# pixray/pixray

Hardware: AMD Instinct MI355X
Metric: optimisation iters/sec, VQGAN 256^2 + ViT-B/32 + 64 cutouts (higher is better)
Workload: dtype fp16

## Files before the change

pixray_amd/csrc/common.h:

```cpp
#pragma once
#include <hip/hip_runtime.h>
#include <stdint.h>

typedef __bf16 bf16_t;
typedef _Float16 half_t;
typedef __attribute__((ext_vector_type(8))) _Float16 f16x8;
typedef __attribute__((ext_vector_type(4))) _Float16 f16x4;
typedef __attribute__((ext_vector_type(8))) __bf16 bf16x8;
typedef __attribute__((ext_vector_type(4))) __bf16 bf16x4;
typedef __attribute__((ext_vector_type(2))) __bf16 bf16x2;
typedef __attribute__((ext_vector_type(16))) float f32x16;
typedef __attribute__((ext_vector_type(4))) float f32x4;

#define PRX_WAVE 64

enum { PRX_PREC_BF16 = 0, PRX_PREC_F32 = 1, PRX_PREC_F16 = 2 };
static inline int prec_is_f32(int precision) { return precision == PRX_PREC_F32; }
static inline int prec_is_h16(int precision) { return precision == PRX_PREC_F16; }
static inline bool prec_valid(int precision) { return precision >= PRX_PREC_BF16 && precision <= PRX_PREC_F16; }
static inline size_t op_esz(int f32) { return f32 ? 4 : 2; }
static inline void* op_off(void* p, size_t elems, int f32) { return p ? (char*)p + elems * op_esz(f32) : nullptr; }
static inline const void* op_off(const void* p, size_t elems, int f32) { return p ? (const char*)p + elems * op_esz(f32) : nullptr; }

void prx_set_error(const char* fmt, ...);
#define PRX_CHECK_HIP(expr)                                                        \
    do {                                                                           \
        hipError_t _e = (expr);                                                    \
        if (_e != hipSuccess) {                                                    \
            prx_set_error("%s:%d: %s -> %s", __FILE__, __LINE__, #expr,            \
                          hipGetErrorString(_e));                                  \
            return -1;                                                             \
        }                                                                          \
    } while (0)
#define PRX_REQUIRE(cond, ...)                                                     \
    do {                                                                           \
        if (!(cond)) {                                                             \
            prx_set_error(__VA_ARGS__);                                            \
            return -2;                                                             \
        }                                                                          \
    } while (0)
#define PRX_LAUNCH_CHECK()                                                         \
    do {                                                                           \
        hipError_t _e = hipGetLastError();                                         \
        if (_e != hipSuccess) {                                                    \
            prx_set_error("%s:%d: kernel launch -> %s", __FILE__, __LINE__,        \
                          hipGetErrorString(_e));                                  \
            return -1;                                                             \
        }                                                                          \
    } while (0)

__device__ __forceinline__ float bf16_to_f32(bf16_t v) { return (float)v; }
__device__ __forceinline__ bf16_t f32_to_bf16(float v) { return (bf16_t)v; }

__device__ __forceinline__ bf16x8 pack_bf16x8(const float* v) {
    bf16x8 r;
#pragma unroll
    for (int i = 0; i < 8; ++i) r[i] = (bf16_t)v[i];
    return r;
}

#define PRX_F16_MAX 65504.f
__device__ __forceinline__ half_t f32_to_f16_sat(float v) {
    return (half_t)__builtin_fminf(__builtin_fmaxf(v, -PRX_F16_MAX), PRX_F16_MAX);
}
__device__ __forceinline__ bf16_t to_op16(float v, int h16) {
    if (h16) return __builtin_bit_cast(bf16_t, f32_to_f16_sat(v));
    return (bf16_t)v;
}
__device__ __forceinline__ float from_op16(bf16_t b, int h16) {
    if (h16) return (float)__builtin_bit_cast(half_t, b);
    return (float)b;
}
__device__ __forceinline__ bf16x4 to_op16x4(float a, float b, float c, float d, int h16) {
    bf16x4 r;
    r[0] = to_op16(a, h16); r[1] = to_op16(b, h16); r[2] = to_op16(c, h16); r[3] = to_op16(d, h16);
    return r;
}

template <bool S16>
__device__ __forceinline__ float4 stream_ld4(const void* p, size_t i4, int h16) {
    if constexpr (S16) {
        const bf16x4 t = reinterpret_cast<const bf16x4*>(p)[i4];
        return make_float4(from_op16(t[0], h16), from_op16(t[1], h16), from_op16(t[2], h16), from_op16(t[3], h16));
    } else {
        return reinterpret_cast<const float4*>(p)[i4];
    }
}

template <typename T> __device__ __forceinline__ float op_ld(const T* p, size_t i) { return (float)p[i]; }
template <typename T> __device__ __forceinline__ void op_st(T* p, size_t i, float v) { p[i] = (T)v; }
template <typename T> __device__ __forceinline__ void op_ld4(const T* p, size_t i, float* v);
template <> __device__ __forceinline__ void op_ld4<bf16_t>(const bf16_t* p, size_t i, float* v) {
    const bf16x4 t = *reinterpret_cast<const bf16x4*>(p + i);
    v[0] = (float)t[0]; v[1] = (float)t[1]; v[2] = (float)t[2]; v[3] = (float)t[3];
}
template <> __device__ __forceinline__ void op_ld4<float>(const float* p, size_t i, float* v) {
    const float4 t = *reinterpret_cast<const float4*>(p + i);
    v[0] = t.x; v[1] = t.y; v[2] = t.z; v[3] = t.w;
}
template <> __device__ __forceinline__ void op_st<half_t>(half_t* p, size_t i, float v) { p[i] = f32_to_f16_sat(v); }
template <> __device__ __forceinline__ void op_ld4<half_t>(const half_t* p, size_t i, float* v) {
    const f16x4 t = *reinterpret_cast<const f16x4*>(p + i);
    v[0] = (float)t[0]; v[1] = (float)t[1]; v[2] = (float)t[2]; v[3] = (float)t[3];
}
template <typename T> __device__ __forceinline__ float4 op_ld4v(const T* p, size_t i);
template <> __device__ __forceinline__ float4 op_ld4v<bf16_t>(const bf16_t* p, size_t i) {
    const bf16x4 t = *reinterpret_cast<const bf16x4*>(p + i);
    return make_float4((float)t[0], (float)t[1], (float)t[2], (float)t[3]);
}
template <> __device__ __forceinline__ float4 op_ld4v<half_t>(const half_t* p, size_t i) {
    const f16x4 t = *reinterpret_cast<const f16x4*>(p + i);
    return make_float4((float)t[0], (float)t[1], (float)t[2], (float)t[3]);
}
template <> __device__ __forceinline__ float4 op_ld4v<float>(const float* p, size_t i) { return *reinterpret_cast<const float4*>(p + i); }
template <typename T> __device__ __forceinline__ void op_st4(T* p, size_t i, float a, float b, float c, float d);
template <> __device__ __forceinline__ void op_st4<half_t>(half_t* p, size_t i, float a, float b, float c, float d) {
    f16x4 r;
    r[0] = f32_to_f16_sat(a); r[1] = f32_to_f16_sat(b); r[2] = f32_to_f16_sat(c); r[3] = f32_to_f16_sat(d);
    *reinterpret_cast<f16x4*>(p + i) = r;
}
template <typename T> __device__ __forceinline__ T op_cvt(float v) { return (T)v; }
template <> __device__ __forceinline__ half_t op_cvt<half_t>(float v) { return f32_to_f16_sat(v); }

#define PRX_OP_DISPATCH(f32_, h16_, T, ...)                                   \
    do {                                                                      \
        if (f32_) { using T = float; __VA_ARGS__; }                           \
        else if (h16_) { using T = half_t; __VA_ARGS__; }                     \
        else { using T = bf16_t; __VA_ARGS__; }                               \
    } while (0)
template <> __device__ __forceinline__ void op_st4<bf16_t>(bf16_t* p, size_t i, float a, float b, float c, float d) {
    bf16x4 r;
    r[0] = (bf16_t)a; r[1] = (bf16_t)b; r[2] = (bf16_t)c; r[3] = (bf16_t)d;
    *reinterpret_cast<bf16x4*>(p + i) = r;
}
template <> __device__ __forceinline__ void op_st4<float>(float* p, size_t i, float a, float b, float c, float d) {
    *reinterpret_cast<float4*>(p + i) = make_float4(a, b, c, d);
}

__device__ __forceinline__ float wave_sum(float v) {
#pragma unroll
    for (int o = 32; o > 0; o >>= 1) v += __shfl_xor(v, o, 64);
    return v;
}
__device__ __forceinline__ float wave_max(float v) {
#pragma unroll
    for (int o = 32; o > 0; o >>= 1) v = fmaxf(v, __shfl_xor(v, o, 64));
    return v;
}
__device__ __forceinline__ float wave_min(float v) {
#pragma unroll
    for (int o = 32; o > 0; o >>= 1) v = fminf(v, __shfl_xor(v, o, 64));
    return v;
}
__device__ __forceinline__ double wave_sum_d(double v) {
#pragma unroll
    for (int o = 32; o > 0; o >>= 1) v += __shfl_xor(v, o, 64);
    return v;
}

__device__ __forceinline__ float sigmoidf_(float x) { return 1.f / (1.f + __expf(-x)); }

__device__ __forceinline__ unsigned xcd_linear(unsigned bid, unsigned nwg) {
    const unsigned xcd = bid & 7u, local = bid >> 3, q = nwg >> 3, r = nwg & 7u;
    return (xcd < r ? xcd * (q + 1) : r * (q + 1) + (xcd - r) * q) + local;
}
int prx_xcd_local();
int prx_grad_target_log2();

static inline int ceil_div(int a, int b) { return (a + b - 1) / b; }
static inline long long ceil_div_ll(long long a, long long b) { return (a + b - 1) / b; }
```

pixray_amd/csrc/elementwise.h:

```cpp
#pragma once
#include "common.h"
int prx_transpose_op(const void* in, int ldin, void* out, int ldout, int R, int C, int f32, hipStream_t s);
int prx_softmax_rows(const float* S, int lds_, float scale, void* P, int ldp, void* PT, int ldpt, int rows,
                     int cols, int prec, hipStream_t s);
int prx_softmax_rows_bwd(const void* P, int ldp, const float* dP, int lddp, float scale, void* dS, int ldds,
                         void* dST, int lddst, int rows, int cols, int prec, hipStream_t s);
int prx_upsample2x_bwd(const void* hi, float* low, bf16_t* low_bf16, int NB, int Hl, int Wl, int C, hipStream_t s, int h16 = 0, int s16 = 0);
int prx_nchw_to_nhwc(const float* in, float* out_f32, bf16_t* out_bf16, int NB, int C, int HW, int Cpad, hipStream_t s, int h16 = 0);
int prx_nhwc_to_nchw(const float* in, int ldc, float* out, int NB, int C, int HW, hipStream_t s);
int prx_image_head_fwd(const float* x, int ldc, float* img, int NB, int C, int HW, hipStream_t s);
int prx_image_head_bwd(const float* x, int ldc, const float* gimg, float* dx, bf16_t* dx_bf16, int ldo, int NB, int C,
                       int HW, hipStream_t s, int h16 = 0, const float* gscale = nullptr);
int prx_image_head_bwd_im2col(const float* x, int ldc, const float* gimg, bf16_t* col, int ldk, int C, int H, int W, hipStream_t s, int h16 = 0,
                              const float* gscale = nullptr);
int prx_grad_scale(const float* g, size_t n, float* part, int nparts, int target_log2, float* scale2, hipStream_t s);
int prx_adam_clamp(float* z, float* m, float* v, const float* g, const float* zmin, const float* zmax, int hw,
                   size_t n, float lr, float b1, float b2, float eps, int step, hipStream_t s);
int prx_adam_clamp_dev(float* z, float* m, float* v, const float* g, const float* zmin, const float* zmax, int hw,
                       size_t n, const float* hyper, float b1, float b2, float eps, hipStream_t s);
int prx_f32_to_bf16(const float* in, bf16_t* out, size_t n, hipStream_t s, int h16 = 0);
int prx_grad_scale_multi(const float* const* gs, const size_t* ns, int count, float* part, int nparts_each, int target_log2,
                         float* scale2, hipStream_t s);
int prx_add_f32(const float* a, const float* b, float* out, size_t n, hipStream_t s);
int prx_scale_dev(float* x, size_t n, const float* scale, hipStream_t s, bf16_t* out16 = nullptr, int h16 = 0);
```

pixray_amd/csrc/elementwise.hip:

```cpp
#include "elementwise.h"
#include <algorithm>

namespace {

inline int ew_grid(size_t total, int per = 256) { return (int)std::min<size_t>((total + per - 1) / per, 8192); }

template <typename T>
__global__ __launch_bounds__(256) void transpose_op_kernel(const T* __restrict__ in, int ldin,
                                                           T* __restrict__ out, int ldout, int R, int C) {
    __shared__ T tile[32][33];
    const int tx = threadIdx.x & 31, ty = threadIdx.x >> 5;
    const int r0 = blockIdx.y * 32, c0 = blockIdx.x * 32;
#pragma unroll
    for (int i = 0; i < 4; ++i) {
        int r = r0 + ty + 8 * i, c = c0 + tx;
        tile[ty + 8 * i][tx] = (r < R && c < C) ? in[(size_t)r * ldin + c] : (T)0.f;
    }
    __syncthreads();
#pragma unroll
    for (int i = 0; i < 4; ++i) {
        int c = c0 + ty + 8 * i, r = r0 + tx;
        if (c < C && r < R) out[(size_t)c * ldout + r] = tile[tx][ty + 8 * i];
    }
}

template <typename T>
__global__ __launch_bounds__(256) void softmax_rows_kernel(const float* __restrict__ S, int lds_, float scale,
                                                           T* __restrict__ P, int ldp, T* __restrict__ PT,
                                                           int ldpt, int rows, int cols) {
    const int lane = threadIdx.x & 63;
    const int row = blockIdx.x * 4 + (threadIdx.x >> 6);
    if (row >= rows) return;
    const float* s = S + (size_t)row * lds_;
    float mx = -INFINITY;
    for (int c = lane; c < cols; c += 64) mx = fmaxf(mx, s[c] * scale);
    mx = wave_max(mx);
    float sum = 0.f;
    for (int c = lane; c < cols; c += 64) sum += __expf(s[c] * scale - mx);
    sum = wave_sum(sum);
    const float inv = 1.f / sum;
    for (int c = lane; c < cols; c += 64) {
        T p = op_cvt<T>(__expf(s[c] * scale - mx) * inv);
        P[(size_t)row * ldp + c] = p;
        if (PT) PT[(size_t)c * ldpt + row] = p;
    }
}

template <typename T>
__global__ __launch_bounds__(256) void softmax_rows_bwd_kernel(const T* __restrict__ P, int ldp,
                                                               const float* __restrict__ dP, int lddp, float scale,
                                                               T* __restrict__ dS, int ldds,
                                                               T* __restrict__ dST, int lddst, int rows, int cols) {
    const int lane = threadIdx.x & 63;
    const int row = blockIdx.x * 4 + (threadIdx.x >> 6);
    if (row >= rows) return;
    float dot = 0.f;
    for (int c = lane; c < cols; c += 64)
        dot += (float)P[(size_t)row * ldp + c] * dP[(size_t)row * lddp + c];
    dot = wave_sum(dot);
    for (int c = lane; c < cols; c += 64) {
        float p = (float)P[(size_t)row * ldp + c];
        T v = op_cvt<T>(scale * p * (dP[(size_t)row * lddp + c] - dot));
        dS[(size_t)row * ldds + c] = v;
        if (dST) dST[(size_t)c * lddst + row] = v;
    }
}

template <bool S16>
__global__ __launch_bounds__(256) void upsample2x_bwd_kernel(const void* __restrict__ hi, float* __restrict__ low,
                                                             bf16_t* __restrict__ low_bf16, int NB, int Hl, int Wl,
                                                             int C, int h16) {
    const int C4 = C >> 2;
    const size_t total = (size_t)NB * Hl * Wl * C4;
    const int Wh = Wl * 2;
    for (size_t idx = (size_t)blockIdx.x * blockDim.x + threadIdx.x; idx < total;
         idx += (size_t)gridDim.x * blockDim.x) {
        int cq = (int)(idx % C4);
        size_t pix = idx / C4;
        int x = (int)(pix % Wl);
        size_t t = pix / Wl;
        int y = (int)(t % Hl);
        int b = (int)(t / Hl);
        size_t p00 = (((size_t)b * Hl * 2 + 2 * y) * Wh + 2 * x) * C4 + cq;
        float4 a = stream_ld4<S16>(hi, p00, h16), bb = stream_ld4<S16>(hi, p00 + C4, h16), c = stream_ld4<S16>(hi, p00 + (size_t)Wh * C4, h16),
               d = stream_ld4<S16>(hi, p00 + (size_t)Wh * C4 + C4, h16);
        float4 o = make_float4((a.x + bb.x) + (c.x + d.x), (a.y + bb.y) + (c.y + d.y), (a.z + bb.z) + (c.z + d.z),
                               (a.w + bb.w) + (c.w + d.w));
        if (low) reinterpret_cast<float4*>(low)[idx] = o;
        if (low_bf16) {
            reinterpret_cast<bf16x4*>(low_bf16)[idx] = to_op16x4(o.x, o.y, o.z, o.w, h16);
        }
    }
}

__global__ __launch_bounds__(256) void nchw_to_nhwc_kernel(const float* __restrict__ in, float* __restrict__ out_f32,
                                                           bf16_t* __restrict__ out_bf16, int NB, int C, int HW,
                                                           int Cpad, int h16) {
    const size_t total = (size_t)NB * HW * Cpad;
    for (size_t idx = (size_t)blockIdx.x * blockDim.x + threadIdx.x; idx < total;
         idx += (size_t)gridDim.x * blockDim.x) {
        int c = (int)(idx % Cpad);
        size_t t = idx / Cpad;
        int p = (int)(t % HW);
        int b = (int)(t / HW);
        float v = c < C ? in[((size_t)b * C + c) * HW + p] : 0.f;
        if (out_f32) out_f32[idx] = v;
        if (out_bf16) out_bf16[idx] = to_op16(v, h16);
    }
}

__global__ __launch_bounds__(256) void nhwc_to_nchw_kernel(const float* __restrict__ in, int ldc,
                                                           float* __restrict__ out, int NB, int C, int HW) {
    const size_t total = (size_t)NB * C * HW;
    for (size_t idx = (size_t)blockIdx.x * blockDim.x + threadIdx.x; idx < total;
         idx += (size_t)gridDim.x * blockDim.x) {
        int p = (int)(idx % HW);
        size_t t = idx / HW;
        int c = (int)(t % C);
        int b = (int)(t / C);
        out[idx] = in[((size_t)b * HW + p) * ldc + c];
    }
}

__global__ __launch_bounds__(256) void image_head_fwd_kernel(const float* __restrict__ x, int ldc,
                                                             float* __restrict__ img, int NB, int C, int HW) {
    const size_t total = (size_t)NB * C * HW;
    for (size_t idx = (size_t)blockIdx.x * blockDim.x + threadIdx.x; idx < total;
         idx += (size_t)gridDim.x * blockDim.x) {
        int p = (int)(idx % HW);
        size_t t = idx / HW;
        int c = (int)(t % C);
        int b = (int)(t / C);
        float v = (x[((size_t)b * HW + p) * ldc + c] + 1.f) * 0.5f;
        img[idx] = fminf(fmaxf(v, 0.f), 1.f);
    }
}

__global__ __launch_bounds__(256) void image_head_bwd_kernel(const float* __restrict__ x, int ldc,
                                                             const float* __restrict__ gimg, float* __restrict__ dx,
                                                             bf16_t* __restrict__ dx_bf16, int ldo, int NB, int C,
                                                             int HW, int h16, const float* __restrict__ gscale_dev) {
    const float gscale = gscale_dev ? *gscale_dev : 1.f;
    const size_t total = (size_t)NB * HW * ldo;
    for (size_t idx = (size_t)blockIdx.x * blockDim.x + threadIdx.x; idx < total;
         idx += (size_t)gridDim.x * blockDim.x) {
        int c = (int)(idx % ldo);
        size_t t = idx / ldo;
        int p = (int)(t % HW);
        int b = (int)(t / HW);
        float o = 0.f;
        if (c < C) {
            float u = (x[((size_t)b * HW + p) * ldc + c] + 1.f) * 0.5f;
            float g = gimg[((size_t)b * C + c) * HW + p];
            float uc = fminf(fmaxf(u, 0.f), 1.f);
            o = (g * (u - uc) >= 0.f) ? (0.5f * gscale) * g : 0.f;
        }
        if (dx) dx[idx] = o;
        if (dx_bf16) dx_bf16[idx] = to_op16(o, h16);
    }
}

__global__ __launch_bounds__(256) void image_head_bwd_im2col_kernel(const float* __restrict__ x, int ldc, const float* __restrict__ gimg,
                                                                    bf16_t* __restrict__ col, int ldk, int C, int H, int W, int h16,
                                                                    const float* __restrict__ gscale_dev) {
    const float gscale = gscale_dev ? *gscale_dev : 1.f;
    const int slots = ldk / 8;
    const size_t HW = (size_t)H * W, total = HW * slots;
    for (size_t idx = (size_t)blockIdx.x * blockDim.x + threadIdx.x; idx < total; idx += (size_t)gridDim.x * blockDim.x) {
        const int tap = (int)(idx % slots);
        const size_t p = idx / slots;
        const int py = (int)(p / W), px = (int)(p - (size_t)py * W);
        bf16x8 o;
#pragma unroll
        for (int c = 0; c < 8; ++c) o[c] = to_op16(0.f, h16);
        if (tap < 9) {
            const int yy = py + tap / 3 - 1, xx = px + tap % 3 - 1;
            if (yy >= 0 && yy < H && xx >= 0 && xx < W) {
                const size_t q = (size_t)yy * W + xx;
#pragma unroll
                for (int c = 0; c < 8; ++c) {
                    if (c < C) {
                        const float u = (x[q * ldc + c] + 1.f) * 0.5f;
                        const float g = gimg[(size_t)c * HW + q];
                        const float uc = fminf(fmaxf(u, 0.f), 1.f);
                        o[c] = to_op16((g * (u - uc) >= 0.f) ? (0.5f * gscale) * g : 0.f, h16);
                    }
                }
            }
        }
        reinterpret_cast<bf16x8*>(col)[idx] = o;
    }
}

__global__ __launch_bounds__(256) void adam_clamp_kernel(float* __restrict__ z, float* __restrict__ m,
                                                         float* __restrict__ v, const float* __restrict__ g,
                                                         const float* __restrict__ zmin, const float* __restrict__ zmax,
                                                         int hw, size_t n, float lr, float b1, float b2, float eps,
                                                         float bc1, float bc2_sqrt, const float* __restrict__ hyper) {
    if (hyper) { lr = hyper[0]; bc1 = 1.f; bc2_sqrt = hyper[1]; }
    for (size_t i = (size_t)blockIdx.x * blockDim.x + threadIdx.x; i < n; i += (size_t)gridDim.x * blockDim.x) {
        float gi = g[i];
        float mi = b1 * m[i] + (1.f - b1) * gi;
        float vi = b2 * v[i] + (1.f - b2) * gi * gi;
        m[i] = mi; v[i] = vi;
        float denom = sqrtf(vi) / bc2_sqrt + eps;
        float zi = z[i] - (lr / bc1) * (mi / denom);
        if (zmin) {
            int c = (int)(i / hw);
            zi = fminf(fmaxf(zi, zmin[c]), zmax[c]);
        }
        z[i] = zi;
    }
}

__global__ __launch_bounds__(256) void f32_to_bf16_kernel(const float* __restrict__ in, bf16_t* __restrict__ out,
                                                          size_t n, int h16) {
    for (size_t i = (size_t)blockIdx.x * blockDim.x + threadIdx.x; i < n; i += (size_t)gridDim.x * blockDim.x)
        out[i] = to_op16(in[i], h16);
}

__global__ __launch_bounds__(256) void amax_partial_kernel(const float* __restrict__ g, size_t n, float* __restrict__ part) {
    float m = 0.f;
    for (size_t i = (size_t)blockIdx.x * blockDim.x + threadIdx.x; i < n; i += (size_t)gridDim.x * blockDim.x) {
        const float a = fabsf(g[i]);
        m = fmaxf(m, a == a ? a : INFINITY);
    }
    m = wave_max(m);
    __shared__ float s[4];
    if ((threadIdx.x & 63) == 0) s[threadIdx.x >> 6] = m;
    __syncthreads();
    if (threadIdx.x == 0) part[blockIdx.x] = fmaxf(fmaxf(s[0], s[1]), fmaxf(s[2], s[3]));
}
__global__ __launch_bounds__(256) void grad_scale_final_kernel(const float* __restrict__ part, int nparts, int target_log2,
                                                               float* __restrict__ scale2) {
    float m = 0.f;
    for (int i = threadIdx.x; i < nparts; i += blockDim.x) m = fmaxf(m, part[i]);
    m = wave_max(m);
    __shared__ float s[4];
    if ((threadIdx.x & 63) == 0) s[threadIdx.x >> 6] = m;
    __syncthreads();
    if (threadIdx.x == 0) {
        m = fmaxf(fmaxf(s[0], s[1]), fmaxf(s[2], s[3]));
        float S = 1.f;
        if (m > 0.f && m < INFINITY) {
            int e;
            (void)frexpf(m, &e);
            int k = target_log2 - e;
            k = k < -40 ? -40 : (k > 60 ? 60 : k);
            S = ldexpf(1.f, k);
        }
        scale2[0] = S;
        scale2[1] = 1.f / S;
    }
}

__global__ __launch_bounds__(256) void scale_dev_kernel(float* __restrict__ x, size_t n, const float* __restrict__ scale, bf16_t* __restrict__ out16, int h16) {
    const float sc = *scale;
    for (size_t i = (size_t)blockIdx.x * blockDim.x + threadIdx.x; i < n; i += (size_t)gridDim.x * blockDim.x) {
        const float v = x[i] * sc;
        x[i] = v;
        if (out16) out16[i] = to_op16(v, h16);
    }
}

__global__ __launch_bounds__(256) void add_f32_kernel(const float* __restrict__ a, const float* __restrict__ b,
                                                      float* __restrict__ out, size_t n) {
    for (size_t i = (size_t)blockIdx.x * blockDim.x + threadIdx.x; i < n; i += (size_t)gridDim.x * blockDim.x)
        out[i] = a[i] + b[i];
}

}

int prx_transpose_op(const void* in, int ldin, void* out, int ldout, int R, int C, int f32, hipStream_t s) {
    dim3 grid(ceil_div(C, 32), ceil_div(R, 32));
    if (f32) hipLaunchKernelGGL(transpose_op_kernel<float>, grid, dim3(256), 0, s, (const float*)in, ldin, (float*)out, ldout, R, C);
    else     hipLaunchKernelGGL(transpose_op_kernel<bf16_t>, grid, dim3(256), 0, s, (const bf16_t*)in, ldin, (bf16_t*)out, ldout, R, C);
    PRX_LAUNCH_CHECK();
    return 0;
}
int prx_softmax_rows(const float* S, int lds_, float scale, void* P, int ldp, void* PT, int ldpt, int rows,
                     int cols, int prec, hipStream_t s) {
    PRX_OP_DISPATCH(prec_is_f32(prec), prec_is_h16(prec), T,
                    hipLaunchKernelGGL(softmax_rows_kernel<T>, dim3(ceil_div(rows, 4)), dim3(256), 0, s, S, lds_, scale, (T*)P, ldp,
                                       (T*)PT, ldpt, rows, cols));
    PRX_LAUNCH_CHECK();
    return 0;
}
int prx_softmax_rows_bwd(const void* P, int ldp, const float* dP, int lddp, float scale, void* dS, int ldds,
                         void* dST, int lddst, int rows, int cols, int prec, hipStream_t s) {
    PRX_OP_DISPATCH(prec_is_f32(prec), prec_is_h16(prec), T,
                    hipLaunchKernelGGL(softmax_rows_bwd_kernel<T>, dim3(ceil_div(rows, 4)), dim3(256), 0, s, (const T*)P, ldp, dP, lddp,
                                       scale, (T*)dS, ldds, (T*)dST, lddst, rows, cols));
    PRX_LAUNCH_CHECK();
    return 0;
}
int prx_upsample2x_bwd(const void* hi, float* low, bf16_t* low_bf16, int NB, int Hl, int Wl, int C, hipStream_t s, int h16, int s16) {
    PRX_REQUIRE(C % 4 == 0 && (low || low_bf16), "upsample2x_bwd: C %% 4 != 0, or no output");
    if (s16) hipLaunchKernelGGL(upsample2x_bwd_kernel<true>, dim3(ew_grid((size_t)NB * Hl * Wl * C / 4)), dim3(256), 0, s, hi, low, low_bf16,
                                NB, Hl, Wl, C, h16);
    else hipLaunchKernelGGL(upsample2x_bwd_kernel<false>, dim3(ew_grid((size_t)NB * Hl * Wl * C / 4)), dim3(256), 0, s, hi, low, low_bf16,
                            NB, Hl, Wl, C, h16);
    PRX_LAUNCH_CHECK();
    return 0;
}
int prx_nchw_to_nhwc(const float* in, float* out_f32, bf16_t* out_bf16, int NB, int C, int HW, int Cpad,
                     hipStream_t s, int h16) {
    hipLaunchKernelGGL(nchw_to_nhwc_kernel, dim3(ew_grid((size_t)NB * HW * Cpad)), dim3(256), 0, s, in, out_f32,
                       out_bf16, NB, C, HW, Cpad, h16);
    PRX_LAUNCH_CHECK();
    return 0;
}
int prx_nhwc_to_nchw(const float* in, int ldc, float* out, int NB, int C, int HW, hipStream_t s) {
    hipLaunchKernelGGL(nhwc_to_nchw_kernel, dim3(ew_grid((size_t)NB * HW * C)), dim3(256), 0, s, in, ldc, out, NB, C,
                       HW);
    PRX_LAUNCH_CHECK();
    return 0;
}
int prx_image_head_fwd(const float* x, int ldc, float* img, int NB, int C, int HW, hipStream_t s) {
    hipLaunchKernelGGL(image_head_fwd_kernel, dim3(ew_grid((size_t)NB * HW * C)), dim3(256), 0, s, x, ldc, img, NB, C,
                       HW);
    PRX_LAUNCH_CHECK();
    return 0;
}
int prx_grad_scale(const float* g, size_t n, float* part, int nparts, int target_log2, float* scale2, hipStream_t s) {
    PRX_REQUIRE(nparts >= 1 && nparts <= 1024, "grad_scale: 1..1024 partials");
    const int blocks = (int)std::min<size_t>((n + 1023) / 1024 + 1, (size_t)nparts);
    hipLaunchKernelGGL(amax_partial_kernel, dim3(blocks), dim3(256), 0, s, g, n, part);
    PRX_LAUNCH_CHECK();
    hipLaunchKernelGGL(grad_scale_final_kernel, dim3(1), dim3(256), 0, s, part, blocks, target_log2, scale2);
    PRX_LAUNCH_CHECK();
    return 0;
}
int prx_grad_scale_multi(const float* const* gs, const size_t* ns, int count, float* part, int nparts_each, int target_log2,
                         float* scale2, hipStream_t s) {
    PRX_REQUIRE(count >= 1 && nparts_each >= 1 && (long long)count * nparts_each <= 4096, "grad_scale_multi: bad partial layout");
    int used = 0;
    for (int i = 0; i < count; ++i) {
        if (!gs[i] || ns[i] == 0) continue;
        const int blocks = (int)std::min<size_t>((ns[i] + 1023) / 1024 + 1, (size_t)nparts_each);
        hipLaunchKernelGGL(amax_partial_kernel, dim3(blocks), dim3(256), 0, s, gs[i], ns[i], part + used);
        PRX_LAUNCH_CHECK();
        used += blocks;
    }
    PRX_REQUIRE(used > 0, "grad_scale_multi: no gradient tensor");
    hipLaunchKernelGGL(grad_scale_final_kernel, dim3(1), dim3(256), 0, s, part, used, target_log2, scale2);
    PRX_LAUNCH_CHECK();
    return 0;
}
int prx_scale_dev(float* x, size_t n, const float* scale, hipStream_t s, bf16_t* out16, int h16) {
    hipLaunchKernelGGL(scale_dev_kernel, dim3(ew_grid(n)), dim3(256), 0, s, x, n, scale, out16, h16);
    PRX_LAUNCH_CHECK();
    return 0;
}
int prx_image_head_bwd(const float* x, int ldc, const float* gimg, float* dx, bf16_t* dx_bf16, int ldo, int NB, int C,
                       int HW, hipStream_t s, int h16, const float* gscale) {
    hipLaunchKernelGGL(image_head_bwd_kernel, dim3(ew_grid((size_t)NB * HW * ldo)), dim3(256), 0, s, x, ldc, gimg, dx,
                       dx_bf16, ldo, NB, C, HW, h16, gscale);
    PRX_LAUNCH_CHECK();
    return 0;
}
int prx_image_head_bwd_im2col(const float* x, int ldc, const float* gimg, bf16_t* col, int ldk, int C, int H, int W, hipStream_t s, int h16,
                              const float* gscale) {
    PRX_REQUIRE(C <= 8 && ldk % 8 == 0 && ldk >= 72, "image_head_bwd_im2col: at most 8 channels, row pitch a multiple of 8 >= 72");
    hipLaunchKernelGGL(image_head_bwd_im2col_kernel, dim3(ew_grid((size_t)H * W * (ldk / 8))), dim3(256), 0, s, x, ldc, gimg, col, ldk, C, H, W,
                       h16, gscale);
    PRX_LAUNCH_CHECK();
    return 0;
}
int prx_adam_clamp(float* z, float* m, float* v, const float* g, const float* zmin, const float* zmax, int hw,
                   size_t n, float lr, float b1, float b2, float eps, int step, hipStream_t s) {
    PRX_REQUIRE(step >= 1, "adam: step must be >= 1");
    const double bc1 = 1.0 - pow((double)b1, step);
    const double bc2 = 1.0 - pow((double)b2, step);
    hipLaunchKernelGGL(adam_clamp_kernel, dim3(ew_grid(n)), dim3(256), 0, s, z, m, v, g, zmin, zmax, hw, n, lr, b1, b2,
                       eps, (float)bc1, (float)sqrt(bc2), (const float*)nullptr);
    PRX_LAUNCH_CHECK();
    return 0;
}
int prx_adam_clamp_dev(float* z, float* m, float* v, const float* g, const float* zmin, const float* zmax, int hw,
                       size_t n, const float* hyper, float b1, float b2, float eps, hipStream_t s) {
    PRX_REQUIRE(hyper != nullptr, "adam: null hyper buffer");
    hipLaunchKernelGGL(adam_clamp_kernel, dim3(ew_grid(n)), dim3(256), 0, s, z, m, v, g, zmin, zmax, hw, n, 0.f, b1, b2,
                       eps, 1.f, 1.f, hyper);
    PRX_LAUNCH_CHECK();
    return 0;
}
int prx_f32_to_bf16(const float* in, bf16_t* out, size_t n, hipStream_t s, int h16) {
    hipLaunchKernelGGL(f32_to_bf16_kernel, dim3(ew_grid(n)), dim3(256), 0, s, in, out, n, h16);
    PRX_LAUNCH_CHECK();
    return 0;
}
int prx_add_f32(const float* a, const float* b, float* out, size_t n, hipStream_t s) {
    hipLaunchKernelGGL(add_f32_kernel, dim3(ew_grid(n)), dim3(256), 0, s, a, b, out, n);
    PRX_LAUNCH_CHECK();
    return 0;
}
```

pixray_amd/csrc/resnet.hip:

```cpp
#include "resnet.h"
#include "gemm.h"
#include "attention.h"
#include "elementwise.h"
#include "cutouts.h"
#include "prompt_vq.h"
#include "vit.h"
#include "dev_arena.h"
#include <cstdlib>
#include <vector>
#include <memory>
#include <algorithm>

namespace {

__constant__ float r_clip_mean[3] = {0.48145466f, 0.4578275f, 0.40821073f};
__constant__ float r_clip_std[3] = {0.26862954f, 0.26130258f, 0.27577711f};

inline int rgrid(size_t total) { return (int)std::min<size_t>((total + 255) / 256, 16384); }

template <typename TOp>
__global__ __launch_bounds__(256) void rn_pack_conv3x3_kernel(const float* __restrict__ w, void* __restrict__ Wf_, void* __restrict__ Wd_,
                                                              int Cout, int Cin) {
    TOp* Wf = reinterpret_cast<TOp*>(Wf_);
    TOp* Wd = reinterpret_cast<TOp*>(Wd_);
    const size_t total = (size_t)Cout * 9 * Cin;
    for (size_t i = (size_t)blockIdx.x * blockDim.x + threadIdx.x; i < 2 * total; i += (size_t)gridDim.x * blockDim.x) {
        if (i < total) {
            const int ci = (int)(i % Cin), tap = (int)((i / Cin) % 9), co = (int)(i / ((size_t)9 * Cin));
            Wf[i] = op_cvt<TOp>(w[(((size_t)co * Cin + ci) * 3 + tap / 3) * 3 + tap % 3]);
        } else {
            const size_t j = i - total;
            const int co = (int)(j % Cout), tap = (int)((j / Cout) % 9), ci = (int)(j / ((size_t)9 * Cout));
            Wd[j] = op_cvt<TOp>(w[(((size_t)co * Cin + ci) * 3 + (2 - tap / 3)) * 3 + (2 - tap % 3)]);
        }
    }
}

template <typename TOp, int CO>
__global__ __launch_bounds__(256) void stem1_fwd_kernel(const float* __restrict__ cut, const float* __restrict__ mm,
                                                        const float* __restrict__ w, const float* __restrict__ b,
                                                        void* __restrict__ out_, int N, int S) {
    __shared__ __attribute__((aligned(16))) float ws[27 * CO];
    __shared__ float bs[CO];
    for (int i = threadIdx.x; i < 27 * CO; i += 256) {
        const int co = i % CO, t = i / CO;
        ws[i] = w[co * 27 + t];
    }
    for (int i = threadIdx.x; i < CO; i += 256) bs[i] = b[i];
    __syncthreads();
    TOp* out = reinterpret_cast<TOp*>(out_);
    const int So = S / 2;
    const float mn = mm[0], range = mm[1] - mm[0];
    const float inv = range != 0.f ? 1.f / range : 1.f;
    const size_t total = (size_t)N * So * So;
    constexpr bool STAGE = sizeof(TOp) == 2;
    __shared__ __attribute__((aligned(16))) TOp otile[STAGE ? 256 * CO : 4];
    for (size_t pixb = (size_t)blockIdx.x * blockDim.x; pixb < total; pixb += (size_t)gridDim.x * blockDim.x) {
        const size_t pix = pixb + threadIdx.x;
        if (pix < total) {
        const int xo = (int)(pix % So), yo = (int)((pix / So) % So), n = (int)(pix / ((size_t)So * So));
        float v[27];
#pragma unroll
        for (int c = 0; c < 3; ++c) {
            const float im = r_clip_mean[c], is = 1.f / r_clip_std[c];
#pragma unroll
            for (int ky = 0; ky < 3; ++ky)
#pragma unroll
                for (int kx = 0; kx < 3; ++kx) {
                    const int y = 2 * yo + ky - 1, x = 2 * xo + kx - 1, t = (c * 3 + ky) * 3 + kx;
                    const bool ok = y >= 0 && y < S && x >= 0 && x < S;
                    const int yc = y < 0 ? 0 : (y < S ? y : S - 1), xc = x < 0 ? 0 : (x < S ? x : S - 1);
                    const float raw = cut[(((size_t)n * 3 + c) * S + yc) * S + xc];
                    v[t] = ok ? ((raw - mn) * inv - im) * is : 0.f;
                }
        }
        TOp* orow = STAGE ? otile + threadIdx.x * CO : out + pix * CO;
#pragma unroll 1
        for (int c0 = 0; c0 < CO; c0 += 4) {
            float a[4] = {bs[c0], bs[c0 + 1], bs[c0 + 2], bs[c0 + 3]};
#pragma unroll
            for (int t = 0; t < 27; ++t) {
                const float4 w4 = *reinterpret_cast<const float4*>(&ws[t * CO + c0]);
                a[0] += v[t] * w4.x; a[1] += v[t] * w4.y; a[2] += v[t] * w4.z; a[3] += v[t] * w4.w;
            }
            op_st4(orow, (size_t)c0, fmaxf(a[0], 0.f), fmaxf(a[1], 0.f), fmaxf(a[2], 0.f), fmaxf(a[3], 0.f));
        }
        }
        if constexpr (STAGE) {
        __syncthreads();
        {
            const size_t pix0 = pixb;
            const size_t npix = total - pix0 < 256 ? total - pix0 : 256;
            const int pieces = (int)(npix * CO * sizeof(TOp) / 16);
            const float4* src = reinterpret_cast<const float4*>(otile);
            float4* dst = reinterpret_cast<float4*>(out + pix0 * CO);
            for (int i = threadIdx.x; i < pieces; i += 256) dst[i] = src[i];
        }
        __syncthreads();
        }
    }
}

template <typename TOp, int CO>
__global__ __launch_bounds__(256) void stem1_bwd_kernel(const void* __restrict__ g_, const float* __restrict__ w, float* __restrict__ dY,
                                                        int N, int S, const float* __restrict__ oscale_dev) {
    const float oscale = oscale_dev ? *oscale_dev : 1.f;
    __shared__ float ws[27 * CO];
    for (int i = threadIdx.x; i < 27 * CO; i += 256) {
        const int co = i % CO, c = (i / CO) % 3, kx = (i / (3 * CO)) % 3, ky = i / (9 * CO);
        ws[i] = w[((co * 3 + c) * 3 + ky) * 3 + kx];
    }
    __syncthreads();
    const TOp* g = reinterpret_cast<const TOp*>(g_);
    const int So = S / 2;
    const size_t plane = (size_t)S * S, total = (size_t)N * plane;
    for (size_t pix = (size_t)blockIdx.x * blockDim.x + threadIdx.x; pix < total; pix += (size_t)gridDim.x * blockDim.x) {
        const int x = (int)(pix % S), y = (int)((pix / S) % S), n = (int)(pix / plane);
        float acc[3] = {0.f, 0.f, 0.f};
        for (int ky = 0; ky < 3; ++ky) {
            const int t = y + 1 - ky;
            if (t < 0 || (t & 1)) continue;
            const int yo = t >> 1;
            if (yo >= So) continue;
            for (int kx = 0; kx < 3; ++kx) {
                const int u = x + 1 - kx;
                if (u < 0 || (u & 1)) continue;
                const int xo = u >> 1;
                if (xo >= So) continue;
                const TOp* gp = g + (((size_t)n * So + yo) * So + xo) * CO;
                const float* wp = ws + (ky * 3 + kx) * 3 * CO;
#pragma unroll
                for (int c0 = 0; c0 < CO; c0 += 4) {
                    float gv[4];
                    op_ld4(gp, (size_t)c0, gv);
#pragma unroll
                    for (int q = 0; q < 4; ++q) {
                        acc[0] += gv[q] * wp[c0 + q];
                        acc[1] += gv[q] * wp[CO + c0 + q];
                        acc[2] += gv[q] * wp[2 * CO + c0 + q];
                    }
                }
            }
        }
        float* o = dY + (size_t)n * 3 * plane + (size_t)y * S + x;
        o[0] = acc[0] * oscale; o[plane] = acc[1] * oscale; o[2 * plane] = acc[2] * oscale;
    }
}

template <typename TOp>
__global__ __launch_bounds__(256) void avgpool2_fwd_kernel(const void* __restrict__ x_, void* __restrict__ out_, int N, int H, int W, int C) {
    const TOp* x = reinterpret_cast<const TOp*>(x_);
    TOp* out = reinterpret_cast<TOp*>(out_);
    const int Ho = H / 2, Wo = W / 2, C4 = C / 4;
    const size_t total = (size_t)N * Ho * Wo * C4;
    for (size_t idx = (size_t)blockIdx.x * blockDim.x + threadIdx.x; idx < total; idx += (size_t)gridDim.x * blockDim.x) {
        const int c = (int)(idx % C4) * 4;
        const size_t pix = idx / C4;
        const int xo = (int)(pix % Wo), yo = (int)((pix / Wo) % Ho), n = (int)(pix / ((size_t)Ho * Wo));
        const size_t p = (((size_t)n * H + 2 * yo) * W + 2 * xo) * C + c;
        const float4 a = op_ld4v(x, p), b = op_ld4v(x, p + C), e = op_ld4v(x, p + (size_t)W * C), f = op_ld4v(x, p + (size_t)W * C + C);
        op_st4(out, pix * C + c, 0.25f * ((a.x + b.x) + (e.x + f.x)), 0.25f * ((a.y + b.y) + (e.y + f.y)),
               0.25f * ((a.z + b.z) + (e.z + f.z)), 0.25f * ((a.w + b.w) + (e.w + f.w)));
    }
}
template <typename TOp>
__global__ __launch_bounds__(256) void avgpool2_bwd_kernel(const float* __restrict__ g, const void* __restrict__ mask_,
                                                           float* __restrict__ dx_f32, void* __restrict__ dx_bf_, int N, int H, int W, int C) {
    const TOp* mask = reinterpret_cast<const TOp*>(mask_);
    TOp* dx_bf = reinterpret_cast<TOp*>(dx_bf_);
    const int Ho = H / 2, Wo = W / 2, C4 = C / 4;
    const size_t total = (size_t)N * Ho * Wo * C4;
    for (size_t idx = (size_t)blockIdx.x * blockDim.x + threadIdx.x; idx < total; idx += (size_t)gridDim.x * blockDim.x) {
        const int c = (int)(idx % C4) * 4;
        const size_t pix = idx / C4;
        const int xo = (int)(pix % Wo), yo = (int)((pix / Wo) % Ho), n = (int)(pix / ((size_t)Ho * Wo));
        float4 v = *reinterpret_cast<const float4*>(g + pix * C + c);
        v.x *= 0.25f; v.y *= 0.25f; v.z *= 0.25f; v.w *= 0.25f;
#pragma unroll
        for (int q = 0; q < 4; ++q) {
            const size_t o = (((size_t)n * H + 2 * yo + (q >> 1)) * W + 2 * xo + (q & 1)) * C + c;
            float4 u = v;
            if (mask) {
                const float4 m = op_ld4v(mask, o);
                if (!(m.x > 0.f)) u.x = 0.f;
                if (!(m.y > 0.f)) u.y = 0.f;
                if (!(m.z > 0.f)) u.z = 0.f;
                if (!(m.w > 0.f)) u.w = 0.f;
            }
            if (dx_f32) *reinterpret_cast<float4*>(dx_f32 + o) = u;
            if (dx_bf) op_st4(dx_bf, o, u.x, u.y, u.z, u.w);
        }
    }
}
template <typename TOp>
__global__ __launch_bounds__(256) void relu_mask_kernel(float* __restrict__ g, const void* __restrict__ out_, void* __restrict__ g_bf_, size_t n) {
    const TOp* out = reinterpret_cast<const TOp*>(out_);
    TOp* g_bf = reinterpret_cast<TOp*>(g_bf_);
    for (size_t i = (size_t)blockIdx.x * blockDim.x + threadIdx.x; i < n; i += (size_t)gridDim.x * blockDim.x) {
        const float v = ((float)out[i] > 0.f) ? g[i] : 0.f;
        g[i] = v;
        g_bf[i] = op_cvt<TOp>(v);
    }
}
template <typename TOp>
__global__ __launch_bounds__(256) void tokens_fwd_kernel(const float* __restrict__ x, const float* __restrict__ pos, void* __restrict__ t_,
                                                         int N, int P, int C) {
    TOp* t = reinterpret_cast<TOp*>(t_);
    const size_t total = (size_t)N * C;
    for (size_t idx = (size_t)blockIdx.x * blockDim.x + threadIdx.x; idx < total; idx += (size_t)gridDim.x * blockDim.x) {
        const int c = (int)(idx % C), n = (int)(idx / C);
        const float* xp = x + (size_t)n * P * C + c;
        TOp* tp = t + (size_t)n * (P + 1) * C + c;
        float sum = 0.f;
        for (int p = 0; p < P; ++p) {
            const float v = xp[(size_t)p * C];
            sum += v;
            tp[(size_t)(p + 1) * C] = op_cvt<TOp>(v + pos[(size_t)(p + 1) * C + c]);
        }
        tp[0] = op_cvt<TOp>(sum / (float)P + pos[c]);
    }
}
template <typename TOp>
__global__ __launch_bounds__(256) void tokens_bwd_kernel(const float* __restrict__ dt, float* __restrict__ dx, int N, int P, int C) {

    const size_t total = (size_t)N * P * C;
    const float ip = 1.f / (float)P;
    for (size_t idx = (size_t)blockIdx.x * blockDim.x + threadIdx.x; idx < total; idx += (size_t)gridDim.x * blockDim.x) {
        const int c = (int)(idx % C);
        const size_t np = idx / C;
        const int p = (int)(np % P), n = (int)(np / P);
        const float* base = dt + (size_t)n * (P + 1) * C + c;
        dx[idx] = base[(size_t)(p + 1) * C] + base[0] * ip;
    }
}
template <typename TOp>
__global__ __launch_bounds__(256) void tok0_gather_kernel(const void* __restrict__ t_, void* __restrict__ out_, int N, int T, int C) {
    const TOp* t = reinterpret_cast<const TOp*>(t_);
    TOp* out = reinterpret_cast<TOp*>(out_);
    const size_t total = (size_t)N * C;
    for (size_t idx = (size_t)blockIdx.x * blockDim.x + threadIdx.x; idx < total; idx += (size_t)gridDim.x * blockDim.x)
        out[idx] = t[(idx / C) * (size_t)T * C + idx % C];
}
template <typename TOp>
__global__ __launch_bounds__(256) void tok0_scatter_kernel(const void* __restrict__ g0_, void* __restrict__ dt_, int N, int T, int C) {
    const TOp* g0 = reinterpret_cast<const TOp*>(g0_);
    TOp* dt = reinterpret_cast<TOp*>(dt_);
    const size_t total = (size_t)N * T * C;
    for (size_t idx = (size_t)blockIdx.x * blockDim.x + threadIdx.x; idx < total; idx += (size_t)gridDim.x * blockDim.x) {
        const int c = (int)(idx % C);
        const size_t nt = idx / C;
        const int tok = (int)(nt % T), n = (int)(nt / T);
        dt[idx] = tok == 0 ? g0[(size_t)n * C + c] : (TOp)0.f;
    }
}

struct RConv1 { int Cin, Cout; void *W, *WT; float* b; };
struct RConv3 { int Cin, Cout; void *Wf, *Wd; float* b; };
struct RBlock {
    int Cin, planes, Hin, stride; bool has_ds;
    RConv1 c1, c3, ds; RConv3 c2;
    void *a1, *a2, *p2, *xp, *out_bf; float* out_f32;
    const void* xin_bf; const float* xin_f32;
};

}

#define RLAUNCH(prec, kernel, total, ...)                                                                                \
    do {                                                                                                                 \
        PRX_REQUIRE(prec_valid(prec), #kernel ": unknown precision %d", prec);                                           \
        PRX_OP_DISPATCH(prec_is_f32(prec), prec_is_h16(prec), TO_,                                                       \
                        hipLaunchKernelGGL(kernel<TO_>, dim3(rgrid(total)), dim3(256), 0, s, __VA_ARGS__));              \
        PRX_LAUNCH_CHECK();                                                                                              \
    } while (0)
#define STEM_CASE(prec, kernel, CO_, total, ...)                                                                         \
    case CO_:                                                                                                            \
        PRX_OP_DISPATCH(prec_is_f32(prec), prec_is_h16(prec), TO_,                                                       \
                        hipLaunchKernelGGL((kernel<TO_, CO_>), dim3(rgrid(total)), dim3(256), 0, s, __VA_ARGS__));       \
        break;
#define STEM_LAUNCH(prec, kernel, total, co, ...)                                                                        \
    do {                                                                                                                 \
        PRX_REQUIRE(prec_valid(prec), #kernel ": unknown precision %d", prec);                                           \
        switch (co) {                                                                                                    \
            STEM_CASE(prec, kernel, 8, total, __VA_ARGS__) STEM_CASE(prec, kernel, 16, total, __VA_ARGS__)               \
            STEM_CASE(prec, kernel, 32, total, __VA_ARGS__) STEM_CASE(prec, kernel, 40, total, __VA_ARGS__)              \
            STEM_CASE(prec, kernel, 48, total, __VA_ARGS__) STEM_CASE(prec, kernel, 64, total, __VA_ARGS__)              \
            default: PRX_REQUIRE(false, "resnet stem: width/2 = %d is not one of 8, 16, 32, 40, 48, 64", co);            \
        }                                                                                                                \
        PRX_LAUNCH_CHECK();                                                                                              \
    } while (0)

int prx_rn_pack_conv3x3(const float* w, void* Wf, void* Wd, int Cout, int Cin, int prec, hipStream_t s) {
    RLAUNCH(prec, rn_pack_conv3x3_kernel, (size_t)1024 * 256, w, Wf, Wd, Cout, Cin);
    return 0;
}
int prx_stem1_fwd(const float* cut, const float* mm, const float* w, const float* b, void* out, int N, int S, int CO, int prec,
                  hipStream_t s) {
    PRX_REQUIRE(N >= 1 && S >= 2, "resnet stem: %d cutouts of side %d", N, S);
    STEM_LAUNCH(prec, stem1_fwd_kernel, (size_t)N * (S / 2) * (S / 2), CO, cut, mm, w, b, out, N, S);
    return 0;
}
int prx_stem1_bwd(const void* g, const float* w, float* dY, int N, int S, int CO, const float* oscale_dev, int prec, hipStream_t s) {
    PRX_REQUIRE(N >= 1 && S >= 2, "resnet stem: %d cutouts of side %d", N, S);
    STEM_LAUNCH(prec, stem1_bwd_kernel, (size_t)N * S * S, CO, g, w, dY, N, S, oscale_dev);
    return 0;
}
int prx_avgpool2_fwd(const void* x, void* out, int N, int H, int W, int C, int prec, hipStream_t s) {
    PRX_REQUIRE(C % 4 == 0, "avgpool2: C = %d is not a multiple of 4", C);
    RLAUNCH(prec, avgpool2_fwd_kernel, (size_t)N * (H / 2) * (W / 2) * C / 4, x, out, N, H, W, C);
    return 0;
}
int prx_avgpool2_bwd(const float* g, const void* mask, float* dx_f32, void* dx_op, int N, int H, int W, int C, int prec, hipStream_t s) {
    PRX_REQUIRE(C % 4 == 0, "avgpool2: C = %d is not a multiple of 4", C);
    RLAUNCH(prec, avgpool2_bwd_kernel, (size_t)N * (H / 2) * (W / 2) * C / 4, g, mask, dx_f32, dx_op, N, H, W, C);
    return 0;
}
int prx_relu_mask(float* g, const void* out, void* g_op, size_t n, int prec, hipStream_t s) {
    RLAUNCH(prec, relu_mask_kernel, n, g, out, g_op, n);
    return 0;
}
int prx_tokens_fwd(const float* x, const float* pos, void* t, int N, int P, int C, int prec, hipStream_t s) {
    RLAUNCH(prec, tokens_fwd_kernel, (size_t)N * C, x, pos, t, N, P, C);
    return 0;
}
int prx_tokens_bwd(const float* dt, float* dx, int N, int P, int C, int prec, hipStream_t s) {
    RLAUNCH(prec, tokens_bwd_kernel, (size_t)N * P * C, dt, dx, N, P, C);
    return 0;
}
int prx_tok0_gather(const void* t, void* out, int N, int T, int C, int prec, hipStream_t s) {
    RLAUNCH(prec, tok0_gather_kernel, (size_t)N * C, t, out, N, T, C);
    return 0;
}
int prx_tok0_scatter(const void* g0, void* dt, int N, int T, int C, int prec, hipStream_t s) {
    RLAUNCH(prec, tok0_scatter_kernel, (size_t)N * T * C, g0, dt, N, T, C);
    return 0;
}

struct PrxResNet {
    int res, width, heads, out_dim, max_n, C, G, T, cur_n;
    int prec;
    int f32, h16;
    int lean;
    float* gs;
    GemmCtx gctx;
    DevArena mem;
    float *w1, *b1;
    RConv3 s2, s3;
    std::vector<RBlock> blocks;
    float* pos; void *Win, *WinT, *Wc, *WcT; float *bin, *bc;
    void *s1, *s2a, *s3a, *s0_bf; float* s0_f32;
    void *tok, *qkv, *att, *o0, *dtok, *dqkv, *do0; float *lse, *e, *de, *dtokf;
    float *gA, *gB, *tf; void *tb1, *tb2, *gbf;
    void *gb2, *gb3;
    float *dY, *mm_part, *ws; size_t ws_bytes;
};

namespace {
struct RCur { const float* const* w; int n, pos; };
#define RNEXT(cur, dst) do { PRX_REQUIRE((cur).pos < (cur).n, "resnet_create: weight list too short"); (dst) = (cur).w[(cur).pos++]; } while (0)

int mk1(PrxResNet* r, RConv1& c, int Cin, int Cout, RCur& cur, hipStream_t s) {
    const float *w, *b; RNEXT(cur, w); RNEXT(cur, b);
    c.Cin = Cin; c.Cout = Cout;
    DEV_ALLOC(r->mem, alloc_op, c.W, (size_t)Cout * Cin, r->f32); DEV_ALLOC(r->mem, alloc_op, c.WT, (size_t)Cout * Cin, r->f32);
    int e;
    if ((e = prx_pack_op(w, c.W, (size_t)Cout * Cin, r->prec, s))) return e;
    if ((e = prx_pack_transpose_op(w, c.WT, Cout, Cin, r->prec, s))) return e;
    return r->mem.copy_f32(&c.b, b, Cout, s);
}
int mk3(PrxResNet* r, RConv3& c, int Cin, int Cout, RCur& cur, hipStream_t s) {
    const float *w, *b; RNEXT(cur, w); RNEXT(cur, b);
    c.Cin = Cin; c.Cout = Cout;
    DEV_ALLOC(r->mem, alloc_op, c.Wf, (size_t)Cout * 9 * Cin, r->f32); DEV_ALLOC(r->mem, alloc_op, c.Wd, (size_t)Cout * 9 * Cin, r->f32);
    int e;
    if ((e = prx_rn_pack_conv3x3(w, c.Wf, c.Wd, Cout, Cin, r->prec, s))) return e;
    return r->mem.copy_f32(&c.b, b, Cout, s);
}
int rg(PrxResNet* r, GemmDesc& d, hipStream_t s) {
    if (r->f32) { d.f32 = 1; d.a_is_f32 = 0; }
    d.h16 = r->h16;
    return prx_gemm_launch(d, r->ws, r->ws_bytes, s, &r->gctx);
}

int lin(PrxResNet* r, const void* A, int M, int K, const void* Bt, int N, const float* bias, const float* resid, int act,
        const void* aux, float* of, void* ob, hipStream_t s, int resid16 = 0) {
    GemmDesc d; d.A = A; d.lda = K; d.B = Bt; d.ldb = K; d.M = M; d.N = N; d.K = K;
    d.bias_n = bias; d.resid = resid; d.ldr = N; d.act = act; d.aux = aux; d.ldaux = N; d.row16 = resid16 ? 1 : 0;
    d.out_f32 = of; d.ldc_f32 = N; d.out_bf16 = ob; d.ldc_bf16 = N;
    return rg(r, d, s);
}
int conv3(PrxResNet* r, const void* x, int NB, int H, int Cin, const void* Bt, int Cout, const float* bias, int act,
          const void* aux, float* of, void* ob, hipStream_t s) {
    GemmDesc d; d.A = x; d.a_mode = PRX_A_CONV3X3; d.lda = Cin; d.B = Bt; d.ldb = 9 * Cin; d.M = NB * H * H; d.N = Cout; d.K = 9 * Cin;
    d.H = H; d.W = H; d.Cin = Cin; d.bias_n = bias; d.act = act; d.aux = aux; d.ldaux = Cout;
    d.out_f32 = of; d.ldc_f32 = Cout; d.out_bf16 = ob; d.ldc_bf16 = Cout;
    return rg(r, d, s);
}
}

GemmCtx* prx_resnet_gemm_ctx_impl(PrxResNet* r) { return r ? &r->gctx : nullptr; }

int prx_resnet_create_impl(PrxResNet** out, int res, int width, const int* layers, int heads, int out_dim, int max_n,
                           int precision, const float* const* w, int n_w, hipStream_t s) {
    PRX_REQUIRE(prec_valid(precision), "resnet_create: unknown precision %d", precision);
    PRX_REQUIRE(res % 32 == 0 && width % 16 == 0 && max_n >= 1, "resnet_create: unsupported geometry (res %d width %d)", res, width);
    PRX_REQUIRE(width * 32 == heads * 64, "resnet_create: the attention pool needs head dim 64 (width %d heads %d)", width, heads);
    std::unique_ptr<PrxResNet> guard(new PrxResNet());
    PrxResNet* r = guard.get();
    DevArena& m = r->mem;
    const int f32 = prec_is_f32(precision);
    m.describe("resnet_create", ": the runner keeps one forward's activations for max_batch = %d cutouts of %d x %d (width %d)", max_n, res, res,
               width);
    r->prec = precision; r->f32 = prec_is_f32(precision); r->h16 = prec_is_h16(precision);
    r->gs = nullptr;
    { const char* ev = getenv("PRX_RN_LEAN"); r->lean = (r->h16 && !(ev && atoi(ev) == 0)) ? 1 : 0; }
    r->res = res; r->width = width; r->heads = heads; r->out_dim = out_dim; r->max_n = max_n; r->cur_n = 0;
    r->C = width * 32; r->G = res / 32; r->T = r->G * r->G + 1;
    RCur cur{w, n_w, 0};
    int e;
    {   const float *ww, *bb; RNEXT(cur, ww); RNEXT(cur, bb);
        if ((e = m.copy_f32(&r->w1, ww, (size_t)(width / 2) * 27, s))) return e;
        if ((e = m.copy_f32(&r->b1, bb, width / 2, s))) return e; }
    if ((e = mk3(r, r->s2, width / 2, width / 2, cur, s))) return e;
    if ((e = mk3(r, r->s3, width / 2, width, cur, s))) return e;
    const size_t N = (size_t)max_n;
    int H = res / 4, inplanes = width;
    size_t maxMC = N * (size_t)(res / 2) * (res / 2) * width;
    for (int li = 0; li < 4; ++li) {
        const int planes = width << li;
        for (int b = 0; b < layers[li]; ++b) {
            RBlock k{};
            k.Cin = inplanes; k.planes = planes; k.Hin = H; k.stride = (li > 0 && b == 0) ? 2 : 1;
            k.has_ds = k.stride > 1 || inplanes != planes * 4;
            if ((e = mk1(r, k.c1, inplanes, planes, cur, s))) return e;
            if ((e = mk3(r, k.c2, planes, planes, cur, s))) return e;
            if ((e = mk1(r, k.c3, planes, planes * 4, cur, s))) return e;
            if (k.has_ds && (e = mk1(r, k.ds, inplanes, planes * 4, cur, s))) return e;
            const size_t Min = N * H * H, Ho = H / k.stride, Mout = N * Ho * Ho;
            DEV_ALLOC(m, alloc_op, k.a1, Min * planes, f32); DEV_ALLOC(m, alloc_op, k.a2, Min * planes, f32);
            k.p2 = k.a2; k.xp = nullptr;
            if (k.stride > 1) { DEV_ALLOC(m, alloc_op, k.p2, Mout * planes, f32); DEV_ALLOC(m, alloc_op, k.xp, Mout * inplanes, f32); }
            DEV_ALLOC(m, alloc_op, k.out_bf, Mout * planes * 4, f32);
            k.out_f32 = nullptr;
            if (!r->lean || (li == 3 && b == layers[li] - 1)) DEV_ALLOC(m, alloc, k.out_f32, Mout * planes * 4);
            maxMC = std::max(maxMC, std::max(Min * (size_t)std::max(inplanes, planes), Mout * (size_t)planes * 4));
            r->blocks.push_back(k);
            inplanes = planes * 4; H = (int)Ho;
        }
    }
    PRX_REQUIRE(inplanes == r->C && H == r->G, "resnet_create: internal geometry mismatch");
    const float *pos, *win, *bin, *wc, *bc;
    RNEXT(cur, pos); RNEXT(cur, win); RNEXT(cur, bin); RNEXT(cur, wc); RNEXT(cur, bc);
    PRX_REQUIRE(cur.pos == n_w, "resnet_create: %d weight tensors given, %d consumed", n_w, cur.pos);
    const int C = r->C, T = r->T;
    if ((e = m.copy_f32(&r->pos, pos, (size_t)T * C, s))) return e;
    DEV_ALLOC(m, alloc_op, r->Win, (size_t)3 * C * C, f32); DEV_ALLOC(m, alloc_op, r->WinT, (size_t)3 * C * C, f32);
    if ((e = prx_pack_op(win, r->Win, (size_t)3 * C * C, r->prec, s))) return e;
    if ((e = prx_pack_transpose_op(win, r->WinT, 3 * C, C, r->prec, s))) return e;
    if ((e = m.copy_f32(&r->bin, bin, 3 * C, s))) return e;
    DEV_ALLOC(m, alloc_op, r->Wc, (size_t)out_dim * C, f32); DEV_ALLOC(m, alloc_op, r->WcT, (size_t)out_dim * C, f32);
    if ((e = prx_pack_op(wc, r->Wc, (size_t)out_dim * C, r->prec, s))) return e;
    if ((e = prx_pack_transpose_op(wc, r->WcT, out_dim, C, r->prec, s))) return e;
    if ((e = m.copy_f32(&r->bc, bc, out_dim, s))) return e;
    const size_t S2 = (size_t)(res / 2) * (res / 2), S4 = (size_t)(res / 4) * (res / 4);
    DEV_ALLOC(m, alloc_op, r->s1, N * S2 * (width / 2), f32); DEV_ALLOC(m, alloc_op, r->s2a, N * S2 * (width / 2), f32);
    DEV_ALLOC(m, alloc_op, r->s3a, N * S2 * width, f32);
    DEV_ALLOC(m, alloc_op, r->s0_bf, N * S4 * width, f32); DEV_ALLOC(m, alloc, r->s0_f32, N * S4 * width);
    DEV_ALLOC(m, alloc_op, r->tok, N * T * C, f32); DEV_ALLOC(m, alloc_op, r->qkv, N * T * 3 * C, f32);
    DEV_ALLOC(m, alloc_op, r->att, N * T * C, f32); DEV_ALLOC(m, alloc_op, r->o0, N * C, f32);
    DEV_ALLOC(m, alloc_op, r->dtok, N * T * C, f32); DEV_ALLOC(m, alloc_op, r->dqkv, N * T * 3 * C, f32); DEV_ALLOC(m, alloc_op, r->do0, N * C, f32);
    DEV_ALLOC(m, alloc, r->dtokf, N * T * C);
    DEV_ALLOC(m, alloc, r->lse, N * heads * T); DEV_ALLOC(m, alloc, r->e, N * out_dim); DEV_ALLOC(m, alloc, r->de, N * out_dim);
    DEV_ALLOC(m, alloc, r->gA, maxMC); DEV_ALLOC(m, alloc, r->tf, maxMC);
    r->gB = nullptr; r->gb2 = r->gb3 = nullptr;
    if (r->lean) { DEV_ALLOC(m, alloc_op, r->gb2, maxMC, f32); DEV_ALLOC(m, alloc_op, r->gb3, maxMC, f32); } else DEV_ALLOC(m, alloc, r->gB, maxMC);
    DEV_ALLOC(m, alloc_op, r->tb1, maxMC, f32); DEV_ALLOC(m, alloc_op, r->tb2, maxMC, f32); DEV_ALLOC(m, alloc_op, r->gbf, maxMC, f32);
    DEV_ALLOC(m, alloc, r->dY, N * 3 * (size_t)res * res); DEV_ALLOC(m, alloc, r->mm_part, 2 * 1024);
    if (r->h16) DEV_ALLOC(m, alloc, r->gs, 2 + 64);
    r->ws_bytes = (size_t)64 << 20;
    DEV_ALLOC(m, alloc, r->ws, r->ws_bytes / sizeof(float));
    *out = guard.release();
    return 0;
}

void prx_resnet_destroy_impl(PrxResNet* r) { delete r; }

int prx_resnet_minmax_impl(PrxResNet* r, const float* cutouts, int n, float* mm, hipStream_t s) {
    PRX_REQUIRE(n >= 1 && n <= r->max_n, "resnet: batch %d exceeds handle capacity %d", n, r->max_n);
    return prx_minmax(cutouts, (size_t)n * 3 * r->res * r->res, r->mm_part, 1024, mm, s);
}

int prx_resnet_forward_impl(PrxResNet* r, const float* cutouts, int n, const float* mm, float* embeds, hipStream_t s) {
    PRX_REQUIRE(n >= 1 && n <= r->max_n, "resnet: batch %d exceeds handle capacity %d", n, r->max_n);
    const int S = r->res, S2 = S / 2, S4 = S / 4, w = r->width, wh = w / 2;
    int e;
    r->cur_n = n;
    if ((e = prx_stem1_fwd(cutouts, mm, r->w1, r->b1, r->s1, n, S, wh, r->prec, s))) return e;
    if ((e = conv3(r, r->s1, n, S2, wh, r->s2.Wf, wh, r->s2.b, PRX_ACT_RELU, nullptr, nullptr, r->s2a, s))) return e;
    if ((e = conv3(r, r->s2a, n, S2, wh, r->s3.Wf, w, r->s3.b, PRX_ACT_RELU, nullptr, nullptr, r->s3a, s))) return e;
    if ((e = prx_avgpool2_fwd(r->s3a, r->s0_bf, n, S2, S2, w, r->prec, s))) return e;
    const void* x_bf = r->s0_bf; const float* x_f32 = nullptr;
    const int lean = r->lean;
    for (RBlock& k : r->blocks) {
        const int H = k.Hin, Ho = H / k.stride, Min = n * H * H, Mout = n * Ho * Ho, p = k.planes;
        k.xin_bf = x_bf; k.xin_f32 = x_f32;
        if ((e = lin(r, x_bf, Min, k.Cin, k.c1.W, p, k.c1.b, nullptr, PRX_ACT_RELU, nullptr, nullptr, k.a1, s))) return e;
        if ((e = conv3(r, k.a1, n, H, p, k.c2.Wf, p, k.c2.b, PRX_ACT_RELU, nullptr, nullptr, k.a2, s))) return e;
        if (k.stride > 1) {
            if ((e = prx_avgpool2_fwd(k.a2, k.p2, n, H, H, p, r->prec, s))) return e;
        }
        const float* idn = lean ? (const float*)x_bf : x_f32;
        if (k.has_ds) {
            const void* xi = x_bf;
            if (k.stride > 1) {
                if ((e = prx_avgpool2_fwd(x_bf, k.xp, n, H, H, k.Cin, r->prec, s))) return e;
                xi = k.xp;
            }
            if ((e = lin(r, xi, Mout, k.Cin, k.ds.W, 4 * p, k.ds.b, nullptr, PRX_ACT_NONE, nullptr, lean ? nullptr : r->tf,
                         lean ? r->tb1 : nullptr, s))) return e;
            idn = lean ? (const float*)r->tb1 : r->tf;
        }
        PRX_REQUIRE(idn != nullptr, "resnet: identity path without an fp32 input");
        if ((e = lin(r, k.p2, Mout, p, k.c3.W, 4 * p, k.c3.b, idn, PRX_ACT_RELU, nullptr, k.out_f32, k.out_bf, s, lean))) return e;
        x_bf = k.out_bf; x_f32 = k.out_f32;
    }
    const int C = r->C, T = r->T, P = T - 1;
    if ((e = prx_tokens_fwd(x_f32, r->pos, r->tok, n, P, C, r->prec, s))) return e;
    if ((e = lin(r, r->tok, n * T, C, r->Win, 3 * C, r->bin, nullptr, PRX_ACT_NONE, nullptr, nullptr, r->qkv, s))) return e;
    if (r->f32) { if ((e = prx_mha_fwd_f32((const float*)r->qkv, (float*)r->att, r->lse, n, T, C, r->heads, s))) return e; }
    else if ((e = prx_mha_fwd_gen((const bf16_t*)r->qkv, (bf16_t*)r->att, r->lse, n, T, C, r->heads, s, r->h16))) return e;
    if ((e = prx_tok0_gather(r->att, r->o0, n, T, C, r->prec, s))) return e;
    if ((e = lin(r, r->o0, n, C, r->Wc, r->out_dim, r->bc, nullptr, PRX_ACT_NONE, nullptr, r->e, nullptr, s))) return e;
    return prx_l2norm_fwd(r->e, embeds, n, r->out_dim, s);
}

int prx_resnet_backward_a_impl(PrxResNet* r, const float* cutouts, const float* mm, const float* d_embeds, double* acc,
                               hipStream_t s) {
    const int n = r->cur_n;
    PRX_REQUIRE(n >= 1, "resnet backward: no forward in flight on this handle");
    const int C = r->C, T = r->T, P = T - 1;
    int e;
    if ((e = prx_l2norm_bwd(r->e, d_embeds, r->de, n, r->out_dim, s))) return e;
    {   GemmDesc d; d.A = r->de; d.a_is_f32 = 1; d.lda = r->out_dim; d.B = r->WcT; d.ldb = r->out_dim; d.M = n; d.N = C; d.K = r->out_dim;
        d.out_bf16 = r->do0; d.ldc_bf16 = C;
        if (r->h16) {
            if ((e = prx_grad_scale(r->de, (size_t)n * r->out_dim, r->gs + 2, 64, prx_grad_target_log2(), r->gs, s))) return e;
            if ((e = prx_scale_dev(r->de, (size_t)n * r->out_dim, r->gs, s))) return e;
        }
        if ((e = rg(r, d, s))) return e; }
    if ((e = prx_tok0_scatter(r->do0, r->dtok, n, T, C, r->prec, s))) return e;
    if (r->f32) { if ((e = prx_mha_bwd_f32((const float*)r->qkv, (const float*)r->att, (const float*)r->dtok, r->lse, (float*)r->dqkv, n, T, C, r->heads, s))) return e; }
    else if ((e = prx_mha_bwd_gen((const bf16_t*)r->qkv, (const bf16_t*)r->att, (const bf16_t*)r->dtok, r->lse, (bf16_t*)r->dqkv, n, T, C, r->heads, s, r->h16))) return e;
    if ((e = lin(r, r->dqkv, n * T, 3 * C, r->WinT, C, nullptr, nullptr, PRX_ACT_NONE, nullptr, r->dtokf, nullptr, s))) return e;
    float* g = r->gA; float* g2 = r->gB;
    const int lean = r->lean;
    void* gb = r->gbf; void* gb_alt = r->gb2;
    if ((e = prx_tokens_bwd(r->dtokf, g, n, P, C, r->prec, s))) return e;
    for (int bi = (int)r->blocks.size() - 1; bi >= 0; --bi) {
        RBlock& k = r->blocks[bi];
        const int H = k.Hin, Ho = H / k.stride, Min = n * H * H, Mout = n * Ho * Ho, p = k.planes;
        if (bi == (int)r->blocks.size() - 1 && (e = prx_relu_mask(g, k.out_bf, gb, (size_t)Mout * 4 * p, r->prec, s))) return e;
        if (k.stride > 1) {
            if ((e = lin(r, gb, Mout, 4 * p, k.c3.WT, p, nullptr, nullptr, PRX_ACT_NONE, nullptr, r->tf, nullptr, s))) return e;
            if ((e = prx_avgpool2_bwd(r->tf, k.a2, nullptr, r->tb1, n, H, H, p, r->prec, s))) return e;
        } else {
            if ((e = lin(r, gb, Mout, 4 * p, k.c3.WT, p, nullptr, nullptr, PRX_ACT_MUL_RELUMASK, k.a2, nullptr, r->tb1, s))) return e;
        }
        if ((e = conv3(r, r->tb1, n, H, p, k.c2.Wd, p, nullptr, PRX_ACT_MUL_RELUMASK, k.a1, nullptr, r->tb2, s))) return e;
        const float* gid = lean ? (const float*)gb : g;
        if (k.has_ds) {
            if (k.stride > 1) {
                if ((e = lin(r, gb, Mout, 4 * p, k.ds.WT, k.Cin, nullptr, nullptr, PRX_ACT_NONE, nullptr, r->tf, nullptr, s))) return e;
                if ((e = prx_avgpool2_bwd(r->tf, nullptr, lean ? (float*)nullptr : g2, lean ? r->gb3 : (void*)nullptr, n, H, H, k.Cin,
                                          r->prec, s))) return e;
                gid = lean ? (const float*)r->gb3 : g2;
            } else {
                if ((e = lin(r, gb, Mout, 4 * p, k.ds.WT, k.Cin, nullptr, nullptr, PRX_ACT_NONE, nullptr, lean ? nullptr : r->tf,
                             lean ? r->gb3 : nullptr, s))) return e;
                gid = lean ? (const float*)r->gb3 : r->tf;
            }
        }
        if (lean) {
            if (bi > 0) {
                if ((e = lin(r, r->tb2, Min, p, k.c1.WT, k.Cin, nullptr, gid, PRX_ACT_RELUMASK_POST, r->blocks[bi - 1].out_bf, nullptr,
                             gb_alt, s, 1))) return e;
                std::swap(gb, gb_alt);
            } else if ((e = lin(r, r->tb2, Min, p, k.c1.WT, k.Cin, nullptr, gid, PRX_ACT_NONE, nullptr, g, nullptr, s, 1))) return e;
            continue;
        }
        float* dst = (gid == g2) ? g : g2;
        if (gid == r->tf) dst = g2;
        if (bi > 0) {
            if ((e = lin(r, r->tb2, Min, p, k.c1.WT, k.Cin, nullptr, gid, PRX_ACT_RELUMASK_POST, r->blocks[bi - 1].out_bf, dst, gb, s))) return e;
        } else if ((e = lin(r, r->tb2, Min, p, k.c1.WT, k.Cin, nullptr, gid, PRX_ACT_NONE, nullptr, dst, nullptr, s))) return e;
        if (dst != g) std::swap(g, g2);
    }
    const int S = r->res, S2 = S / 2, w = r->width, wh = w / 2;
    if ((e = prx_avgpool2_bwd(g, r->s3a, nullptr, r->tb1, n, S2, S2, w, r->prec, s))) return e;
    if ((e = conv3(r, r->tb1, n, S2, w, r->s3.Wd, wh, nullptr, PRX_ACT_MUL_RELUMASK, r->s2a, nullptr, r->tb2, s))) return e;
    if ((e = conv3(r, r->tb2, n, S2, wh, r->s2.Wd, wh, nullptr, PRX_ACT_MUL_RELUMASK, r->s1, nullptr, r->tb1, s))) return e;
    if ((e = prx_stem1_bwd(r->tb1, r->w1, r->dY, n, S, wh, r->h16 ? r->gs + 1 : nullptr, r->prec, s))) return e;
    return prx_preproc_bwd_reduce(cutouts, mm, r->dY, acc, n, S, s);
}

int prx_resnet_backward_b_impl(PrxResNet* r, const float* cutouts, const float* mm, const double* acc, float* g_cutouts,
                               hipStream_t s) {
    PRX_REQUIRE(r->cur_n >= 1, "resnet backward: no forward in flight on this handle");
    return prx_preproc_bwd_apply(cutouts, mm, r->dY, acc, g_cutouts, r->cur_n, r->res, s);
}
```

pixray_amd/csrc/vit.hip:

```cpp
#include "vit.h"
#include <stdlib.h>
#include "gemm.h"
#include "norms.h"
#include "attention.h"
#include "cutouts.h"
#include "prompt_vq.h"
#include "elementwise.h"
#include "dev_arena.h"
#include <vector>
#include <memory>

namespace {

template <typename TOp>
__global__ __launch_bounds__(256) void pack_transpose_kernel(const float* __restrict__ in, TOp* __restrict__ out,
                                                             int R, int C) {
    __shared__ float tile[32][33];
    const int tx = threadIdx.x & 31, ty = threadIdx.x >> 5;
    const int r0 = blockIdx.y * 32, c0 = blockIdx.x * 32;
#pragma unroll
    for (int i = 0; i < 4; ++i) {
        int r = r0 + ty + 8 * i, c = c0 + tx;
        tile[ty + 8 * i][tx] = (r < R && c < C) ? in[(size_t)r * C + c] : 0.f;
    }
    __syncthreads();
#pragma unroll
    for (int i = 0; i < 4; ++i) {
        int c = c0 + ty + 8 * i, r = r0 + tx;
        if (c < C && r < R) out[(size_t)c * R + r] = op_cvt<TOp>(tile[tx][ty + 8 * i]);
    }
}

__global__ __launch_bounds__(256) void add_cls_pos_kernel(float* __restrict__ x, const float* __restrict__ cls,
                                                          const float* __restrict__ pos, int N, int T, int W) {
    const size_t total = (size_t)N * T * W;
    for (size_t i = (size_t)blockIdx.x * blockDim.x + threadIdx.x; i < total; i += (size_t)gridDim.x * blockDim.x) {
        const int c = (int)(i % W);
        const int t = (int)((i / W) % T);
        float v = x[i] + pos[(size_t)t * W + c];
        if (t == 0) v += cls[c];
        x[i] = v;
    }
}

template <typename TOut>
__global__ __launch_bounds__(256) void embed_tokens_kernel(const float* __restrict__ x, const float* __restrict__ cls,
                                                           const float* __restrict__ pos, TOut* __restrict__ out, int N, int T, int W) {
    const size_t total = (size_t)N * T * W;
    for (size_t i = (size_t)blockIdx.x * blockDim.x + threadIdx.x; i < total; i += (size_t)gridDim.x * blockDim.x) {
        const int c = (int)(i % W);
        const int t = (int)((i / W) % T);
        const float p = pos[(size_t)t * W + c];
        op_st(out, i, t == 0 ? cls[c] + p : x[i] + p);
    }
}

__global__ __launch_bounds__(256) void scale_f32_kernel(float* __restrict__ x, size_t n, float s) {
    for (size_t i = (size_t)blockIdx.x * blockDim.x + threadIdx.x; i < n; i += (size_t)gridDim.x * blockDim.x) x[i] *= s;
}

template <bool BWD>
__global__ __launch_bounds__(256) void gelu_f32_kernel(const float* __restrict__ t, float* __restrict__ io, size_t n) {
    for (size_t i = (size_t)blockIdx.x * blockDim.x + threadIdx.x; i < n; i += (size_t)gridDim.x * blockDim.x) {
        const float x = t[i];
        const float cdf = 0.5f * (1.f + erff(x * 0.70710678f));
        if (BWD) io[i] *= cdf + x * (0.39894228f * expf(-0.5f * x * x));
        else io[i] = x * cdf;
    }
}

}

int prx_pack_op(const float* in, void* out, size_t n, int prec, hipStream_t s) {
    if (!prec_is_f32(prec)) return prx_f32_to_bf16(in, (bf16_t*)out, n, s, prec_is_h16(prec));
    PRX_CHECK_HIP(hipMemcpyAsync(out, in, n * sizeof(float), hipMemcpyDeviceToDevice, s));
    return 0;
}
int prx_pack_transpose_op(const float* in, void* out, int R, int C, int prec, hipStream_t s) {
    const dim3 grid(ceil_div(C, 32), ceil_div(R, 32));
    PRX_OP_DISPATCH(prec_is_f32(prec), prec_is_h16(prec), TO,
                    hipLaunchKernelGGL(pack_transpose_kernel<TO>, grid, dim3(256), 0, s, in, (TO*)out, R, C));
    PRX_LAUNCH_CHECK();
    return 0;
}
int prx_pack_bf16(const float* in, bf16_t* out, size_t n, hipStream_t s) { return prx_pack_op(in, out, n, 0, s); }
int prx_pack_transpose_bf16(const float* in, bf16_t* out, int R, int C, hipStream_t s) { return prx_pack_transpose_op(in, out, R, C, 0, s); }
int prx_vit_add_cls_pos(float* x, const float* cls, const float* pos, int N, int T, int W, hipStream_t s) {
    hipLaunchKernelGGL(add_cls_pos_kernel, dim3(2048), dim3(256), 0, s, x, cls, pos, N, T, W);
    PRX_LAUNCH_CHECK();
    return 0;
}
int prx_vit_embed_tokens(const float* x, const float* cls, const float* pos, void* out, int out16, int N, int T, int W, hipStream_t s) {
    if (out16) hipLaunchKernelGGL(embed_tokens_kernel<half_t>, dim3(2048), dim3(256), 0, s, x, cls, pos, (half_t*)out, N, T, W);
    else hipLaunchKernelGGL(embed_tokens_kernel<float>, dim3(2048), dim3(256), 0, s, x, cls, pos, (float*)out, N, T, W);
    PRX_LAUNCH_CHECK();
    return 0;
}
int prx_vit_gelu_f32(const float* t, float* io, size_t n, int bwd, hipStream_t s) {
    if (bwd) hipLaunchKernelGGL(gelu_f32_kernel<true>, dim3(2048), dim3(256), 0, s, t, io, n);
    else hipLaunchKernelGGL(gelu_f32_kernel<false>, dim3(2048), dim3(256), 0, s, t, io, n);
    PRX_LAUNCH_CHECK();
    return 0;
}
int prx_vit_scale_f32(float* x, size_t n, float scale, int blocks, hipStream_t s) {
    PRX_REQUIRE(blocks >= 1, "scale_f32: %d workgroups", blocks);
    hipLaunchKernelGGL(scale_f32_kernel, dim3(blocks), dim3(256), 0, s, x, n, scale);
    PRX_LAUNCH_CHECK();
    return 0;
}

struct VitLayer {
    float *ln1_g, *ln1_b, *bqkv, *bo, *ln2_g, *ln2_b, *b1, *b2;
    void *Wqkv, *WqkvT, *Wo, *WoT, *W1, *W1T, *W2, *W2T;
    void *x_in, *x_mid;
    float *mean1, *rstd1, *mean2, *rstd2;
    void *qkv, *t;
    void* o_save;
    float* lse;
};

struct PrxVit {
    int res, patch, width, layers, heads, out_dim, T, max_n, KP;
    int hd, aw;
    int prec;
    int f32, h16;
    float* gs;
    GemmCtx gctx;
    DevArena mem;
    void *Wp, *WpT, *projT, *proj;
    float *cls, *pos, *lnpre_g, *lnpre_b, *lnpost_g, *lnpost_b;
    std::vector<VitLayer> L;
    void *A0, *h, *att_o, *u, *hpost, *dt, *do_, *dqkv, *dx_bf, *dh_bf, *de16;
    float *xpre, *mean_pre, *rstd_pre, *mean_post, *rstd_post, *e, *dx, *dh, *dA0, *de, *dhpost, *mm_part;
    void* x_final;
    int lean;
    VitFamily fam;
    float* bp;
    int cls_tail;
    float* ws; size_t ws_bytes;
    int cur_n;
};

namespace {
int pack_both(PrxVit* v, void** W, void** WT, const float* src, int out, int in, hipStream_t s) {
    DEV_ALLOC(v->mem, alloc_op, *W, (size_t)out * in, v->f32);
    DEV_ALLOC(v->mem, alloc_op, *WT, (size_t)out * in, v->f32);
    int r = prx_pack_op(src, *W, (size_t)out * in, v->prec, s);
    if (r) return r;
    return prx_pack_transpose_op(src, *WT, out, in, v->prec, s);
}
}

VitFamily prx_vit_family_clip() {
    VitFamily f;
    f.patch_bias = 0; f.ln_pre = 1; f.eps = 1e-5f; f.act = PRX_ACT_QUICKGELU; f.dact = PRX_ACT_MUL_DQUICKGELU;
    f.norm = prx_patch_norm_clip(); f.head_dim = 64;
    return f;
}

int prx_vit_create_impl(PrxVit** out, int res, int patch, int width, int layers, int heads, int out_dim, int max_n,
                        int precision, const float* const* w, int n_w, hipStream_t s, const VitFamily* family) {
    const VitFamily fam = family ? *family : prx_vit_family_clip();
    const int n_head = 3 + (fam.patch_bias ? 1 : 0) + (fam.ln_pre ? 2 : 0);
    PRX_REQUIRE(prec_valid(precision), "vit_create: unknown precision %d", precision);
    PRX_REQUIRE(n_w == n_head + 12 * layers + 3, "vit_create: expected %d weight tensors, got %d", n_head + 12 * layers + 3, n_w);
    const int hd = fam.head_dim > 0 ? fam.head_dim : 64;
    PRX_REQUIRE(res % patch == 0 && width == heads * hd && width % 128 == 0 && (hd == 64 || hd == 32 || hd == 16),
                "vit_create: unsupported geometry (width %d, %d heads of %d)", width, heads, hd);
    PRX_REQUIRE(fam.ln_pre || layers >= 1, "vit_create: a tower without ln_pre needs at least one block");
    PRX_REQUIRE(fam.eps > 0.f && fam.norm.std[0] > 0.f && fam.norm.std[1] > 0.f && fam.norm.std[2] > 0.f,
                "vit_create: LayerNorm eps and the channel std must be positive");
    const int G = res / patch;
    const int T = G * G + 1;
    std::unique_ptr<PrxVit> guard(new PrxVit());
    PrxVit* v = guard.get();
    DevArena& m = v->mem;
    const int f32 = prec_is_f32(precision);
    v->mem.describe("vit_create", ": the runner keeps one forward's activations for max_batch = %d cutouts of %d tokens (width %d, %d layers)",
                    max_n, T, width, layers);
    v->T = T; v->max_n = max_n;
    v->res = res; v->patch = patch; v->width = width; v->layers = layers; v->heads = heads; v->out_dim = out_dim;
    v->prec = precision; v->f32 = prec_is_f32(precision); v->h16 = prec_is_h16(precision);
    v->gs = nullptr; v->fam = fam; v->bp = nullptr; v->hd = hd; v->aw = heads * 64;
    const int AW = v->aw;
    float *pad_w = nullptr, *pad_b = nullptr;
    if (hd != 64) {
        DEV_ALLOC(m, alloc, pad_w, (size_t)3 * AW * width);
        DEV_ALLOC(m, alloc, pad_b, (size_t)3 * AW);
    }
    { const char* e = getenv("PRX_LEAN"); v->lean = (v->h16 && !(e && atoi(e) == 0)) ? 1 : 0; }
    { const char* e = getenv("PRX_VIT_CLS_TAIL"); v->cls_tail = (e && atoi(e) == 0) ? 0 : 1; }
    v->T = T; v->max_n = max_n; v->KP = (3 * patch * patch + 7) / 8 * 8; v->cur_n = 0;
    const int W = width, KP = v->KP;
    int r;
    {
        const int K0 = 3 * patch * patch;
        float* padded;
        DEV_ALLOC(m, alloc, padded, (size_t)W * KP);
        PRX_CHECK_HIP(hipMemsetAsync(padded, 0, sizeof(float) * (size_t)W * KP, s));
        PRX_CHECK_HIP(hipMemcpy2DAsync(padded, sizeof(float) * KP, w[0], sizeof(float) * K0, sizeof(float) * K0, W,
                                       hipMemcpyDeviceToDevice, s));
        if ((r = pack_both(v, &v->Wp, &v->WpT, padded, W, KP, s))) return r;
    }
    const float* const* wh = w + 1;
    if (fam.patch_bias) { if ((r = v->mem.copy_f32(&v->bp, *wh++, W, s))) return r; }
    if ((r = v->mem.copy_f32(&v->cls, *wh++, W, s))) return r;
    if ((r = v->mem.copy_f32(&v->pos, *wh++, (size_t)T * W, s))) return r;
    v->lnpre_g = v->lnpre_b = nullptr;
    if (fam.ln_pre) {
        if ((r = v->mem.copy_f32(&v->lnpre_g, *wh++, W, s))) return r;
        if ((r = v->mem.copy_f32(&v->lnpre_b, *wh++, W, s))) return r;
    }
    v->L.resize(layers);
    const size_t R = (size_t)max_n * T;
    for (int l = 0; l < layers; ++l) {
        const float* const* q = w + n_head + 12 * l;
        VitLayer& y = v->L[l];
        if ((r = v->mem.copy_f32(&y.ln1_g, q[0], W, s))) return r;
        if ((r = v->mem.copy_f32(&y.ln1_b, q[1], W, s))) return r;
        if (hd == 64) {
            if ((r = pack_both(v, &y.Wqkv, &y.WqkvT, q[2], 3 * W, W, s))) return r;
            if ((r = v->mem.copy_f32(&y.bqkv, q[3], 3 * W, s))) return r;
            if ((r = pack_both(v, &y.Wo, &y.WoT, q[4], W, W, s))) return r;
        } else {
            const float qs = sqrtf(64.f / (float)hd);
            PRX_CHECK_HIP(hipMemsetAsync(pad_w, 0, sizeof(float) * (size_t)3 * AW * W, s));
            PRX_CHECK_HIP(hipMemsetAsync(pad_b, 0, sizeof(float) * (size_t)3 * AW, s));
            for (int sect = 0; sect < 3; ++sect) {
                PRX_CHECK_HIP(hipMemcpy2DAsync(pad_w + (size_t)sect * AW * W, sizeof(float) * 64 * W, q[2] + (size_t)sect * W * W, sizeof(float) * hd * W,
                                               sizeof(float) * hd * W, heads, hipMemcpyDeviceToDevice, s));
                PRX_CHECK_HIP(hipMemcpy2DAsync(pad_b + (size_t)sect * AW, sizeof(float) * 64, q[3] + (size_t)sect * W, sizeof(float) * hd,
                                               sizeof(float) * hd, heads, hipMemcpyDeviceToDevice, s));
            }
            if ((r = prx_vit_scale_f32(pad_w, (size_t)AW * W, qs, 256, s))) return r;
            if ((r = prx_vit_scale_f32(pad_b, (size_t)AW, qs, 1, s))) return r;
            if ((r = pack_both(v, &y.Wqkv, &y.WqkvT, pad_w, 3 * AW, W, s))) return r;
            if ((r = v->mem.copy_f32(&y.bqkv, pad_b, 3 * AW, s))) return r;
            PRX_CHECK_HIP(hipMemsetAsync(pad_w, 0, sizeof(float) * (size_t)W * AW, s));
            PRX_CHECK_HIP(hipMemcpy2DAsync(pad_w, sizeof(float) * 64, q[4], sizeof(float) * hd, sizeof(float) * hd, (size_t)W * heads,
                                           hipMemcpyDeviceToDevice, s));
            if ((r = pack_both(v, &y.Wo, &y.WoT, pad_w, W, AW, s))) return r;
        }
        if ((r = v->mem.copy_f32(&y.bo, q[5], W, s))) return r;
        if ((r = v->mem.copy_f32(&y.ln2_g, q[6], W, s))) return r;
        if ((r = v->mem.copy_f32(&y.ln2_b, q[7], W, s))) return r;
        if ((r = pack_both(v, &y.W1, &y.W1T, q[8], 4 * W, W, s))) return r;
        if ((r = v->mem.copy_f32(&y.b1, q[9], 4 * W, s))) return r;
        if ((r = pack_both(v, &y.W2, &y.W2T, q[10], W, 4 * W, s))) return r;
        if ((r = v->mem.copy_f32(&y.b2, q[11], W, s))) return r;
        if (v->lean) { DEV_ALLOC(m, alloc_op, y.x_in, R * W, f32); DEV_ALLOC(m, alloc_op, y.x_mid, R * W, f32); }
        else { float *a_, *b_; DEV_ALLOC(m, alloc, a_, R * W); DEV_ALLOC(m, alloc, b_, R * W); y.x_in = a_; y.x_mid = b_; }
        DEV_ALLOC(m, alloc, y.mean1, R); DEV_ALLOC(m, alloc, y.rstd1, R); DEV_ALLOC(m, alloc, y.mean2, R); DEV_ALLOC(m, alloc, y.rstd2, R);
        DEV_ALLOC(m, alloc_op, y.qkv, R * 3 * AW, f32); DEV_ALLOC(m, alloc_op, y.t, R * 4 * W, f32);
        y.o_save = nullptr; y.lse = nullptr;
        if (T > 64 || v->f32) { DEV_ALLOC(m, alloc_op, y.o_save, R * AW, f32); DEV_ALLOC(m, alloc, y.lse, (size_t)max_n * heads * T); }
    }
    const float* const* q = w + n_head + 12 * layers;
    if ((r = v->mem.copy_f32(&v->lnpost_g, q[0], W, s))) return r;
    if ((r = v->mem.copy_f32(&v->lnpost_b, q[1], W, s))) return r;
    if ((r = pack_both(v, &v->proj, &v->projT, q[2], W, out_dim, s))) return r;
    DEV_ALLOC(m, alloc_op, v->A0, R * KP, f32); DEV_ALLOC(m, alloc_op, v->h, R * W, f32);
    DEV_ALLOC(m, alloc_op, v->att_o, R * AW, f32); DEV_ALLOC(m, alloc_op, v->u, R * 4 * W, f32);
    DEV_ALLOC(m, alloc_op, v->hpost, (size_t)max_n * W, f32); DEV_ALLOC(m, alloc_op, v->de16, (size_t)max_n * out_dim, f32);
    DEV_ALLOC(m, alloc_op, v->dt, R * 4 * W, f32); DEV_ALLOC(m, alloc_op, v->do_, R * AW, f32); DEV_ALLOC(m, alloc_op, v->dqkv, R * 3 * AW, f32);
    DEV_ALLOC(m, alloc, v->xpre, R * W); DEV_ALLOC(m, alloc, v->mean_pre, R); DEV_ALLOC(m, alloc, v->rstd_pre, R);
    if (v->lean) DEV_ALLOC(m, alloc_op, v->x_final, R * W, f32);
    else { float* a_; DEV_ALLOC(m, alloc, a_, R * W); v->x_final = a_; }
    DEV_ALLOC(m, alloc, v->mean_post, max_n); DEV_ALLOC(m, alloc, v->rstd_post, max_n); DEV_ALLOC(m, alloc, v->e, (size_t)max_n * out_dim);
    v->dx = v->dh = nullptr;
    if (!v->lean) { DEV_ALLOC(m, alloc, v->dx, R * W); DEV_ALLOC(m, alloc, v->dh, R * W); }
    DEV_ALLOC(m, alloc, v->dA0, R * KP); DEV_ALLOC(m, alloc, v->de, (size_t)max_n * out_dim);
    if (v->f32) { v->dx_bf = v->dx; v->dh_bf = v->dh; }
    else { DEV_ALLOC(m, alloc_op, v->dx_bf, R * W, f32); DEV_ALLOC(m, alloc_op, v->dh_bf, R * W, f32); }
    DEV_ALLOC(m, alloc, v->dhpost, (size_t)max_n * W); DEV_ALLOC(m, alloc, v->mm_part, 2 * 1024);
    if (v->h16) DEV_ALLOC(m, alloc, v->gs, 2 + 64);
    v->ws_bytes = (size_t)64 << 20;
    DEV_ALLOC(m, alloc, v->ws, v->ws_bytes / sizeof(float));
    *out = guard.release();
    return 0;
}

void prx_vit_destroy_impl(PrxVit* v) { delete v; }

static int vit_gemm(PrxVit* v, GemmDesc& d, hipStream_t s) {
    if (v->f32) { d.f32 = 1; d.a_is_f32 = 0; }
    d.h16 = v->h16;
    return prx_gemm_launch(d, v->ws, v->ws_bytes, s, &v->gctx);
}
GemmCtx* prx_vit_gemm_ctx_impl(PrxVit* v) { return v ? &v->gctx : nullptr; }
long long prx_vit_debug_dqkv_impl(PrxVit* v, void* dst, long long max_bytes, hipStream_t s) {
    if (!v || v->cur_n < 1) return -1;
    const long long bytes = (long long)op_esz(v->f32) * v->cur_n * v->T * 3 * v->aw;
    if (bytes > max_bytes || hipMemcpyAsync(dst, v->dqkv, bytes, hipMemcpyDeviceToDevice, s) != hipSuccess) return -1;
    return bytes;
}

static int ln_op(PrxVit* v, const void* x, long long ldx, const float* g, const float* b, void* out, float* mean, float* rstd,
                 int rows, hipStream_t s) {
    return prx_layernorm_fwd(x, ldx, g, b, v->f32 ? nullptr : (bf16_t*)out, v->f32 ? (float*)out : nullptr, mean, rstd, rows,
                             v->width, v->fam.eps, s, v->h16, v->lean, 1);
}
static int ln_bwd_op(PrxVit* v, const void* g, long long ldg, const void* x, long long ldx, const float* gamma, const float* mean,
                     const float* rstd, const void* add, long long ldadd, float* dx, long long lddx, void* dx_op, int rows,
                     hipStream_t s, int add_every = 0, int s16 = 0) {
    return prx_layernorm_bwd(g, ldg, x, ldx, gamma, mean, rstd, add, ldadd, dx, lddx, v->f32 ? nullptr : (bf16_t*)dx_op, lddx, rows,
                             v->width, s, v->h16, add_every, s16, 1);
}

int prx_vit_minmax_impl(PrxVit* v, const float* cutouts, int n, float* mm, hipStream_t s) {
    PRX_REQUIRE(n >= 1 && n <= v->max_n, "vit: batch %d exceeds handle capacity %d", n, v->max_n);
    return prx_minmax(cutouts, (size_t)n * 3 * v->res * v->res, v->mm_part, 1024, mm, s);
}

int prx_vit_forward_impl(PrxVit* v, const float* cutouts, int n, const float* mm, float* embeds, hipStream_t s) {
    PRX_REQUIRE(n >= 1 && n <= v->max_n, "vit: batch %d exceeds handle capacity %d", n, v->max_n);
    const int W = v->width, T = v->T, R = n * T, KP = v->KP, AW = v->aw;
    int r;
    v->cur_n = n;
    if ((r = prx_patchify_fwd(cutouts, mm, v->A0, v->prec, n, v->res, v->patch, T, s, v->fam.norm))) return r;
    {
        GemmDesc d; d.A = v->A0; d.lda = KP; d.B = v->Wp; d.ldb = KP; d.M = R; d.N = W; d.K = KP;
        d.bias_n = v->bp;
        d.out_f32 = v->xpre; d.ldc_f32 = W;
        if ((r = vit_gemm(v, d, s))) return r;
    }
    const int lean = v->lean;
    void* x0 = v->layers > 0 ? v->L[0].x_in : v->x_final;
    if (v->fam.ln_pre) {
        if ((r = prx_vit_add_cls_pos(v->xpre, v->cls, v->pos, n, T, W, s))) return r;
        if ((r = prx_layernorm_fwd(v->xpre, W, v->lnpre_g, v->lnpre_b, lean ? (bf16_t*)x0 : nullptr, lean ? nullptr : (float*)x0, v->mean_pre,
                                   v->rstd_pre, R, W, v->fam.eps, s, v->h16, 0, 1))) return r;
    } else {
        if ((r = prx_vit_embed_tokens(v->xpre, v->cls, v->pos, x0, lean, n, T, W, s))) return r;
    }
    for (int l = 0; l < v->layers; ++l) {
        VitLayer& y = v->L[l];
        void* x_next = (l + 1 < v->layers) ? v->L[l + 1].x_in : v->x_final;
        if ((r = ln_op(v, y.x_in, W, y.ln1_g, y.ln1_b, v->h, y.mean1, y.rstd1, R, s))) return r;
        {   GemmDesc d; d.A = v->h; d.lda = W; d.B = y.Wqkv; d.ldb = W; d.M = R; d.N = 3 * AW; d.K = W;
            d.bias_n = y.bqkv; d.out_bf16 = y.qkv; d.ldc_bf16 = 3 * AW;
            if ((r = vit_gemm(v, d, s))) return r; }
        const void* att = v->att_o;
        if (v->f32) { if ((r = prx_mha_fwd_f32((const float*)y.qkv, (float*)y.o_save, y.lse, n, T, AW, v->heads, s))) return r; att = y.o_save; }
        else if (T <= 64) { if ((r = prx_mha_fwd((const bf16_t*)y.qkv, (bf16_t*)v->att_o, n, T, AW, v->heads, s, v->h16))) return r; }
        else { if ((r = prx_mha_fwd_gen((const bf16_t*)y.qkv, (bf16_t*)y.o_save, y.lse, n, T, AW, v->heads, s, v->h16))) return r; att = y.o_save; }
        const bool tail = v->cls_tail && l == v->layers - 1;
        const int rows = tail ? n : R;
        const int ldt = tail ? T * W : W;
        {   GemmDesc d; d.A = att; d.lda = tail ? T * AW : AW; d.B = y.Wo; d.ldb = AW; d.M = rows; d.N = W; d.K = AW;
            d.bias_n = y.bo; d.ldr = ldt;
            if (lean) { d.resid = (const float*)y.x_in; d.row16 = 1; d.out_bf16 = y.x_mid; d.ldc_bf16 = ldt; }
            else { d.resid = (const float*)y.x_in; d.out_f32 = (float*)y.x_mid; d.ldc_f32 = ldt; }
            if ((r = vit_gemm(v, d, s))) return r; }
        if ((r = ln_op(v, y.x_mid, ldt, y.ln2_g, y.ln2_b, v->h, y.mean2, y.rstd2, rows, s))) return r;
        {   GemmDesc d; d.A = v->h; d.lda = W; d.B = y.W1; d.ldb = W; d.M = rows; d.N = 4 * W; d.K = W;
            d.bias_n = y.b1; d.act = v->fam.act; d.out_bf16 = v->u; d.out_bf16_pre = y.t; d.ldc_bf16 = 4 * W;
            const bool own_pass = v->f32 && v->fam.act == PRX_ACT_GELU;
            if (own_pass) { d.act = PRX_ACT_NONE; d.out_bf16 = y.t; d.out_bf16_pre = nullptr; }
            if ((r = vit_gemm(v, d, s))) return r;
            if (own_pass) {
                if ((r = prx_vit_gelu_f32((const float*)y.t, (float*)v->u, (size_t)rows * 4 * W, 0, s))) return r;
            } }
        {   GemmDesc d; d.A = v->u; d.lda = 4 * W; d.B = y.W2; d.ldb = 4 * W; d.M = rows; d.N = W; d.K = 4 * W;
            d.bias_n = y.b2; d.ldr = ldt;
            if (lean) { d.resid = (const float*)y.x_mid; d.row16 = 1; d.out_bf16 = x_next; d.ldc_bf16 = ldt; }
            else { d.resid = (const float*)y.x_mid; d.out_f32 = (float*)x_next; d.ldc_f32 = ldt; }
            if ((r = vit_gemm(v, d, s))) return r; }
    }
    if ((r = ln_op(v, v->x_final, (long long)T * W, v->lnpost_g, v->lnpost_b, v->hpost, v->mean_post, v->rstd_post, n, s))) return r;
    {   GemmDesc d; d.A = v->hpost; d.lda = W; d.B = v->projT; d.ldb = W; d.M = n; d.N = v->out_dim; d.K = W;
        d.out_f32 = v->e; d.ldc_f32 = v->out_dim;
        if ((r = vit_gemm(v, d, s))) return r; }
    return prx_l2norm_fwd(v->e, embeds, n, v->out_dim, s);
}

int prx_vit_backward_a_impl(PrxVit* v, const float* cutouts, const float* mm, const float* d_embeds, double* acc,
                            hipStream_t s) {
    const int n = v->cur_n;
    PRX_REQUIRE(n >= 1, "vit backward: no forward in flight on this handle");
    const int W = v->width, T = v->T, R = n * T, KP = v->KP, AW = v->aw;
    int r;
    if ((r = prx_l2norm_bwd(v->e, d_embeds, v->de, n, v->out_dim, s))) return r;
    {   GemmDesc d; d.A = v->de; d.a_is_f32 = 1; d.lda = v->out_dim; d.B = v->proj; d.ldb = v->out_dim;
        d.M = n; d.N = W; d.K = v->out_dim; d.out_f32 = v->dhpost; d.ldc_f32 = W;
        if (v->h16) {
            if ((r = prx_grad_scale(v->de, (size_t)n * v->out_dim, v->gs + 2, 64, prx_grad_target_log2(), v->gs, s))) return r;
            if ((r = prx_scale_dev(v->de, (size_t)n * v->out_dim, v->gs, s, (bf16_t*)v->de16, v->h16))) return r;
            d.A = v->de16; d.a_is_f32 = 0;
        }
        if ((r = vit_gemm(v, d, s))) return r; }
    const int lean = v->lean;
    if (v->layers == 0 || !v->cls_tail) PRX_CHECK_HIP(hipMemsetAsync(lean ? v->dx_bf : (void*)v->dx, 0, (lean ? sizeof(bf16_t) : sizeof(float)) * (size_t)R * W, s));
    const void* dxs = lean ? v->dx_bf : (const void*)v->dx;
    const void* dhs = lean ? v->dh_bf : (const void*)v->dh;
    if ((r = ln_bwd_op(v, v->dhpost, W, v->x_final, (long long)T * W, v->lnpost_g, v->mean_post, v->rstd_post,
                       nullptr, 0, v->dx, (long long)T * W, v->dx_bf, n, s, 0, lean ? 1 : 0))) return r;
    for (int l = v->layers - 1; l >= 0; --l) {
        VitLayer& y = v->L[l];
        const bool tail = v->cls_tail && l == v->layers - 1;
        const int rows = tail ? n : R;
        const int ldt = tail ? T * W : W;
        {   GemmDesc d; d.A = v->dx_bf; d.lda = ldt; d.B = y.W2T; d.ldb = W; d.M = rows; d.N = 4 * W; d.K = W;
            d.act = v->fam.dact; d.aux = y.t; d.ldaux = 4 * W; d.out_bf16 = v->dt; d.ldc_bf16 = 4 * W;
            const bool own_pass = v->f32 && v->fam.dact == PRX_ACT_MUL_DGELU;
            if (own_pass) { d.act = PRX_ACT_NONE; d.aux = nullptr; }
            if ((r = vit_gemm(v, d, s))) return r;
            if (own_pass) {
                if ((r = prx_vit_gelu_f32((const float*)y.t, (float*)v->dt, (size_t)rows * 4 * W, 1, s))) return r;
            } }
        {   GemmDesc d; d.A = v->dt; d.lda = 4 * W; d.B = y.W1T; d.ldb = 4 * W; d.M = rows; d.N = W; d.K = 4 * W;
            if (lean) { d.out_bf16 = v->dh_bf; d.ldc_bf16 = W; } else { d.out_f32 = v->dh; d.ldc_f32 = W; }
            if ((r = vit_gemm(v, d, s))) return r; }
        if ((r = ln_bwd_op(v, dhs, W, y.x_mid, ldt, y.ln2_g, y.mean2, y.rstd2, dxs, ldt, v->dx, ldt, v->dx_bf, rows, s, 0, lean ? 7 : 0))) return r;
        if (tail)
            PRX_CHECK_HIP(hipMemsetAsync(v->do_, 0, op_esz(v->f32) * (size_t)R * AW, s));
        {   GemmDesc d; d.A = v->dx_bf; d.lda = ldt; d.B = y.WoT; d.ldb = W; d.M = rows; d.N = AW; d.K = W;
            d.out_bf16 = v->do_; d.ldc_bf16 = tail ? T * AW : AW;
            if ((r = vit_gemm(v, d, s))) return r; }
        if (v->f32) { if ((r = prx_mha_bwd_f32((const float*)y.qkv, (const float*)y.o_save, (const float*)v->do_, y.lse, (float*)v->dqkv, n, T, AW, v->heads, s))) return r; }
        else if (T <= 64) { if ((r = prx_mha_bwd((const bf16_t*)y.qkv, (const bf16_t*)v->do_, (bf16_t*)v->dqkv, n, T, AW, v->heads, s, v->h16))) return r; }
        else { if ((r = prx_mha_bwd_gen((const bf16_t*)y.qkv, (const bf16_t*)y.o_save, (const bf16_t*)v->do_, y.lse, (bf16_t*)v->dqkv, n, T, AW, v->heads, s, v->h16))) return r; }
        {   GemmDesc d; d.A = v->dqkv; d.lda = 3 * AW; d.B = y.WqkvT; d.ldb = 3 * AW; d.M = R; d.N = W; d.K = 3 * AW;
            if (lean) { d.out_bf16 = v->dh_bf; d.ldc_bf16 = W; } else { d.out_f32 = v->dh; d.ldc_f32 = W; }
            if ((r = vit_gemm(v, d, s))) return r; }
        if ((r = ln_bwd_op(v, dhs, W, y.x_in, W, y.ln1_g, y.mean1, y.rstd1, dxs, W, v->dx, W, v->dx_bf, R, s, tail ? T : 0, lean ? 7 : 0))) return r;
    }
    if (v->fam.ln_pre) { if ((r = ln_bwd_op(v, dxs, W, v->xpre, W, v->lnpre_g, v->mean_pre, v->rstd_pre, nullptr, 0, v->dh, W, v->dh_bf, R, s, 0, lean ? 2 : 0))) return r; }
    {   GemmDesc d; d.A = v->fam.ln_pre ? v->dh_bf : v->dx_bf; d.lda = W; d.B = v->WpT; d.ldb = W; d.M = R; d.N = KP; d.K = W;
        d.out_f32 = v->dA0; d.ldc_f32 = KP;
        if (v->h16) d.alpha_dev = v->gs + 1;
        if ((r = vit_gemm(v, d, s))) return r; }
    return prx_patchify_bwd_reduce(cutouts, mm, v->dA0, acc, n, v->res, v->patch, T, s, v->fam.norm);
}

int prx_vit_backward_b_impl(PrxVit* v, const float* cutouts, const float* mm, const double* acc, float* g_cutouts,
                            hipStream_t s) {
    const int n = v->cur_n;
    PRX_REQUIRE(n >= 1, "vit backward: no forward in flight on this handle");
    int r = prx_patchify_bwd_apply(cutouts, mm, v->dA0, acc, g_cutouts, n, v->res, v->patch, v->T, s, v->fam.norm);
    return r;
}
```

pixray_amd/csrc/vqgan.hip:

```cpp
#include "vqgan.h"
#include "gemm.h"
#include "norms.h"
#include "elementwise.h"
#include "prompt_vq.h"
#include "vit.h"
#include "dev_arena.h"
#include <vector>
#include <memory>
#include <stdlib.h>

namespace {

template <typename TOp>
__global__ __launch_bounds__(256) void pack_conv3x3_kernel(const float* __restrict__ w, TOp* __restrict__ Wf,
                                                           TOp* __restrict__ Wd, int Cout, int Cin, int CoP) {
    const size_t total_f = (size_t)Cout * 9 * Cin;
    const size_t total_d = (size_t)Cin * 9 * CoP;
    for (size_t i = (size_t)blockIdx.x * blockDim.x + threadIdx.x; i < total_f + total_d;
         i += (size_t)gridDim.x * blockDim.x) {
        if (i < total_f) {
            int ci = (int)(i % Cin);
            int tap = (int)((i / Cin) % 9);
            int co = (int)(i / ((size_t)9 * Cin));
            Wf[i] = op_cvt<TOp>(w[(((size_t)co * Cin + ci) * 3 + tap / 3) * 3 + tap % 3]);
        } else {
            size_t j = i - total_f;
            int co = (int)(j % CoP);
            int tap = (int)((j / CoP) % 9);
            int ci = (int)(j / ((size_t)9 * CoP));
            int ky = 2 - tap / 3, kx = 2 - tap % 3;
            Wd[j] = op_cvt<TOp>((co < Cout) ? w[(((size_t)co * Cin + ci) * 3 + ky) * 3 + kx] : 0.f);
        }
    }
}

__global__ __launch_bounds__(256) void colminmax_kernel(const float* __restrict__ w, float* __restrict__ mn,
                                                        float* __restrict__ mx, int rows, int D) {
    const int c = blockIdx.x * blockDim.x + threadIdx.x;
    if (c >= D) return;
    float a = INFINITY, b = -INFINITY;
    for (int r = 0; r < rows; ++r) { float v = w[(size_t)r * D + c]; a = fminf(a, v); b = fmaxf(b, v); }
    mn[c] = a; mx[c] = b;
}

}

int prx_vqgan_pack_conv3x3(const float* w, void* Wf, void* Wd, int Cout, int Cin, int CoP, int prec, hipStream_t s) {
    PRX_REQUIRE(prec_valid(prec), "vqgan pack_conv3x3: unknown precision %d", prec);
    PRX_OP_DISPATCH(prec_is_f32(prec), prec_is_h16(prec), TO,
                    hipLaunchKernelGGL(pack_conv3x3_kernel<TO>, dim3(1024), dim3(256), 0, s, w, (TO*)Wf, (TO*)Wd, Cout, Cin, CoP));
    PRX_LAUNCH_CHECK();
    return 0;
}
int prx_colminmax(const float* w, float* mn, float* mx, int rows, int D, hipStream_t s) {
    hipLaunchKernelGGL(colminmax_kernel, dim3(ceil_div(D, 256)), dim3(256), 0, s, w, mn, mx, rows, D);
    PRX_LAUNCH_CHECK();
    return 0;
}

static inline int pad8(int P) { return (P + 7) & ~7; }

struct Conv3 { int Cin, Cout, CoP; void *Wf, *Wd; float* b; };
struct Conv1 { int Cin, Cout; void *W, *WT; float* b; };
struct GN { int C; float *g, *b; double *stats, *bstats; int id; };

struct ResBlock {
    int Cin, Cout, rh, rw;
    GN n1, n2; Conv3 c1, c2; Conv1 sc; bool has_sc;
    void *x_in, *h1, *scbuf, *out;
    void *x_in_bf, *out_bf;
};
struct AttnBlock {
    int C, rh, rw;
    GN n; Conv1 qkv, proj;
    void* x_in; void *qkvb, *Pm, *PT; void* out; void* out_bf;
    void* qkvT;
};
struct UpBlock { int C, rh, rw; Conv3 c; void *x_in, *out; void *x_in_bf, *out_bf; };

struct Stage { int kind; int idx; };

struct PrxVqgan {
    int zc, D, NC, ch, out_ch, h0, w0, H, W, nstage;
    int prec;
    int f32, h16;
    int lean;
    float* gs;
    GemmCtx gctx;
    DevArena mem;
    float *codebook, *cnorm, *zmin, *zmax;
    Conv1 pq; Conv3 conv_in, conv_out; GN norm_out;
    std::vector<ResBlock> res; std::vector<AttnBlock> attn; std::vector<UpBlock> ups; std::vector<Stage> stages;
    float *zq, *y, *dzq; void* h_in; int* idx; void *pqo_bf, *h_in_bf, *dpq_bf;
    float *pmin; int* pidx;
    void* a;
    void *tA, *tB, *tC, *tD, *dqkv, *dy8;
    void *dycol, *Wd_col;
    float* S;
    void *g0, *g1, *g2;
    void *g0b, *g1b, *g2b;
    double* all_stats; int n_gn;
    float* ws; size_t ws_bytes;
    void* x_last;
};

namespace {
int alloc_stream(PrxVqgan* v, void** p, size_t count) { return v->mem.alloc_op(p, count, !v->lean); }

struct WCursor { const float* const* w; int n, pos; };
#define NEXTW(cur, dst) do { PRX_REQUIRE((cur).pos < (cur).n, "vqgan_create: weight list too short"); (dst) = (cur).w[(cur).pos++]; } while (0)

int make_gn(PrxVqgan* v, GN& g, int C, WCursor& cur, hipStream_t s) {
    const float *w, *b; NEXTW(cur, w); NEXTW(cur, b);
    g.C = C;
    int r;
    if ((r = v->mem.copy_f32(&g.g, w, C, s))) return r;
    if ((r = v->mem.copy_f32(&g.b, b, C, s))) return r;
    g.id = v->n_gn++;
    g.stats = g.bstats = nullptr;
    return 0;
}
int make_conv3(PrxVqgan* v, Conv3& c, int Cin, int Cout, WCursor& cur, hipStream_t s) {
    const float *w, *b; NEXTW(cur, w); NEXTW(cur, b);
    c.Cin = Cin; c.Cout = Cout; c.CoP = (Cout + 7) / 8 * 8;
    DEV_ALLOC(v->mem, alloc_op, c.Wf, (size_t)c.CoP * 9 * Cin, v->f32);
    if (c.CoP != Cout) PRX_CHECK_HIP(hipMemsetAsync(c.Wf, 0, (size_t)c.CoP * 9 * Cin * op_esz(v->f32), s));
    DEV_ALLOC(v->mem, alloc_op, c.Wd, (size_t)Cin * 9 * c.CoP, v->f32);
    { int e_ = prx_vqgan_pack_conv3x3(w, c.Wf, c.Wd, Cout, Cin, c.CoP, v->prec, s); if (e_) return e_; }
    DEV_ALLOC(v->mem, alloc, c.b, c.CoP);
    if (c.CoP != Cout) PRX_CHECK_HIP(hipMemsetAsync(c.b, 0, sizeof(float) * c.CoP, s));
    PRX_CHECK_HIP(hipMemcpyAsync(c.b, b, sizeof(float) * Cout, hipMemcpyDeviceToDevice, s));
    return 0;
}
int make_conv1(PrxVqgan* v, Conv1& c, int Cin, int Cout, WCursor& cur, hipStream_t s) {
    const float *w, *b; NEXTW(cur, w); NEXTW(cur, b);
    c.Cin = Cin; c.Cout = Cout;
    DEV_ALLOC(v->mem, alloc_op, c.W, (size_t)Cout * Cin, v->f32); DEV_ALLOC(v->mem, alloc_op, c.WT, (size_t)Cout * Cin, v->f32);
    int r;
    if ((r = prx_pack_op(w, c.W, (size_t)Cout * Cin, v->prec, s))) return r;
    if ((r = prx_pack_transpose_op(w, c.WT, Cout, Cin, v->prec, s))) return r;
    return v->mem.copy_f32(&c.b, b, Cout, s);
}
int make_res(PrxVqgan* v, int Cin, int Cout, int rh, int rw, WCursor& cur, hipStream_t s) {
    ResBlock rb{};
    rb.Cin = Cin; rb.Cout = Cout; rb.rh = rh; rb.rw = rw; rb.has_sc = Cin != Cout;
    int r;
    if ((r = make_gn(v, rb.n1, Cin, cur, s))) return r;
    if ((r = make_conv3(v, rb.c1, Cin, Cout, cur, s))) return r;
    if ((r = make_gn(v, rb.n2, Cout, cur, s))) return r;
    if ((r = make_conv3(v, rb.c2, Cout, Cout, cur, s))) return r;
    const size_t P = (size_t)rh * rw;
    if (rb.has_sc) {
        if ((r = make_conv1(v, rb.sc, Cin, Cout, cur, s))) return r;
        if ((r = alloc_stream(v, &rb.scbuf, P * Cout))) return r;
    }
    if ((r = alloc_stream(v, &rb.h1, P * Cout))) return r;
    if ((r = alloc_stream(v, &rb.out, P * Cout))) return r;
    v->stages.push_back({0, (int)v->res.size()});
    v->res.push_back(rb);
    return 0;
}
int make_attn(PrxVqgan* v, int C, int rh, int rw, WCursor& cur, hipStream_t s) {
    AttnBlock ab{};
    ab.C = C; ab.rh = rh; ab.rw = rw;
    int r;
    if ((r = make_gn(v, ab.n, C, cur, s))) return r;
    const float *wq, *bq, *wk, *bk, *wv, *bv;
    NEXTW(cur, wq); NEXTW(cur, bq); NEXTW(cur, wk); NEXTW(cur, bk); NEXTW(cur, wv); NEXTW(cur, bv);
    float *wcat, *bcat;
    DEV_ALLOC(v->mem, alloc, wcat, (size_t)3 * C * C); DEV_ALLOC(v->mem, alloc, bcat, 3 * C);
    const float* ws_[3] = {wq, wk, wv}; const float* bs_[3] = {bq, bk, bv};
    for (int i = 0; i < 3; ++i) {
        PRX_CHECK_HIP(hipMemcpyAsync(wcat + (size_t)i * C * C, ws_[i], sizeof(float) * C * C, hipMemcpyDeviceToDevice, s));
        PRX_CHECK_HIP(hipMemcpyAsync(bcat + i * C, bs_[i], sizeof(float) * C, hipMemcpyDeviceToDevice, s));
    }
    ab.qkv.Cin = C; ab.qkv.Cout = 3 * C; ab.qkv.b = bcat;
    DEV_ALLOC(v->mem, alloc_op, ab.qkv.W, (size_t)3 * C * C, v->f32); DEV_ALLOC(v->mem, alloc_op, ab.qkv.WT, (size_t)3 * C * C, v->f32);
    if ((r = prx_pack_op(wcat, ab.qkv.W, (size_t)3 * C * C, v->prec, s))) return r;
    if ((r = prx_pack_transpose_op(wcat, ab.qkv.WT, 3 * C, C, v->prec, s))) return r;
    if ((r = make_conv1(v, ab.proj, C, C, cur, s))) return r;
    const size_t P = (size_t)rh * rw;
    const size_t P8 = (size_t)pad8((int)P);
    DEV_ALLOC(v->mem, alloc_op, ab.qkvb, P * 3 * C, v->f32);
    DEV_ALLOC(v->mem, alloc_op, ab.Pm, P * P8, v->f32); DEV_ALLOC(v->mem, alloc_op, ab.PT, P * P8, v->f32);
    if ((r = alloc_stream(v, &ab.out, P * C))) return r;
    DEV_ALLOC(v->mem, alloc_op, ab.qkvT, (size_t)3 * C * P8, v->f32);
    PRX_CHECK_HIP(hipMemsetAsync(ab.qkvT, 0, (size_t)3 * C * P8 * op_esz(v->f32), s));
    PRX_CHECK_HIP(hipMemsetAsync(ab.Pm, 0, P * P8 * op_esz(v->f32), s));
    PRX_CHECK_HIP(hipMemsetAsync(ab.PT, 0, P * P8 * op_esz(v->f32), s));
    v->stages.push_back({1, (int)v->attn.size()});
    v->attn.push_back(ab);
    return 0;
}
int make_up(PrxVqgan* v, int C, int rh, int rw, WCursor& cur, hipStream_t s) {
    UpBlock ub{};
    ub.C = C; ub.rh = rh; ub.rw = rw;
    int r;
    if ((r = make_conv3(v, ub.c, C, C, cur, s))) return r;
    if ((r = alloc_stream(v, &ub.out, (size_t)rh * rw * C))) return r;
    v->stages.push_back({2, (int)v->ups.size()});
    v->ups.push_back(ub);
    return 0;
}
}

int prx_vqgan_create_impl(PrxVqgan** out, int ch, const int* ch_mult, int n_mult, int num_res_blocks, int attn_res,
                          int resolution, int z_channels, int embed_dim, int n_embed, int out_ch, int h0, int w0,
                          int precision, const float* const* w, int n_w, hipStream_t s) {
    PRX_REQUIRE(h0 >= 1 && w0 >= 1, "vqgan_create: bad latent size %dx%d", h0, w0);
    PRX_REQUIRE(prec_valid(precision), "vqgan_create: unknown precision %d", precision);
    PRX_REQUIRE(embed_dim == z_channels, "vqgan_create: embed_dim must equal z_channels");
    std::unique_ptr<PrxVqgan> guard(new PrxVqgan());
    PrxVqgan* v = guard.get();
    DevArena& m = v->mem;
    const int f32 = prec_is_f32(precision);
    m.describe("vqgan_create", ": the decoder keeps one forward's activations and the backward's gradient streams for a %d x %d latent", h0, w0);
    v->prec = precision; v->f32 = prec_is_f32(precision); v->h16 = prec_is_h16(precision);
    v->gs = nullptr;
    { const char* e = getenv("PRX_LEAN"); v->lean = (v->h16 && !(e && atoi(e) == 0)) ? 1 : 0; }
    v->n_gn = 0; v->zc = z_channels; v->D = embed_dim; v->NC = n_embed; v->ch = ch; v->out_ch = out_ch; v->h0 = h0; v->w0 = w0;
    WCursor cur{w, n_w, 0};
    int r;
    const float* cb; NEXTW(cur, cb);
    if ((r = m.copy_f32(&v->codebook, cb, (size_t)n_embed * embed_dim, s))) return r;
    DEV_ALLOC(m, alloc, v->cnorm, n_embed); DEV_ALLOC(m, alloc, v->zmin, embed_dim); DEV_ALLOC(m, alloc, v->zmax, embed_dim);
    if ((r = prx_sqnorm_rows(v->codebook, v->cnorm, n_embed, embed_dim, s))) return r;
    if ((r = prx_colminmax(v->codebook, v->zmin, v->zmax, n_embed, embed_dim, s))) return r;
    if ((r = make_conv1(v, v->pq, embed_dim, z_channels, cur, s))) return r;
    int block_in = ch * ch_mult[n_mult - 1];
    int rh = h0, rw = w0;
    if ((r = make_conv3(v, v->conv_in, z_channels, block_in, cur, s))) return r;
    if ((r = make_res(v, block_in, block_in, rh, rw, cur, s))) return r;
    if ((r = make_attn(v, block_in, rh, rw, cur, s))) return r;
    if ((r = make_res(v, block_in, block_in, rh, rw, cur, s))) return r;
    int nominal = resolution >> (n_mult - 1);
    for (int lvl = n_mult - 1; lvl >= 0; --lvl) {
        int block_out = ch * ch_mult[lvl];
        for (int b = 0; b < num_res_blocks + 1; ++b) {
            if ((r = make_res(v, block_in, block_out, rh, rw, cur, s))) return r;
            block_in = block_out;
            if (nominal == attn_res) { if ((r = make_attn(v, block_in, rh, rw, cur, s))) return r; }
        }
        if (lvl != 0) {
            rh *= 2; rw *= 2; nominal *= 2;
            if ((r = make_up(v, block_in, rh, rw, cur, s))) return r;
        }
    }
    v->H = rh; v->W = rw;
    if ((r = make_gn(v, v->norm_out, block_in, cur, s))) return r;
    if ((r = make_conv3(v, v->conv_out, block_in, out_ch, cur, s))) return r;
    PRX_REQUIRE(cur.pos == n_w, "vqgan_create: %d weight tensors given, %d consumed", n_w, cur.pos);
    const size_t P0 = (size_t)h0 * w0, PH = (size_t)rh * rw;
    size_t maxPC = P0 * (size_t)std::max(z_channels, embed_dim), maxAttnPC = 1;
    for (auto& rb : v->res) maxPC = std::max(maxPC, (size_t)rb.rh * rb.rw * std::max(rb.Cin, rb.Cout));
    for (auto& ub : v->ups) maxPC = std::max(maxPC, (size_t)ub.rh * ub.rw * ub.C);
    for (auto& ab : v->attn) maxAttnPC = std::max(maxAttnPC, (size_t)pad8(ab.rh * ab.rw) * (size_t)std::max(ab.C, pad8(ab.rh * ab.rw)));
    DEV_ALLOC(m, alloc, v->zq, P0 * embed_dim); DEV_ALLOC(m, alloc_op, v->pqo_bf, P0 * z_channels, f32);
    DEV_ALLOC(m, alloc_op, v->dpq_bf, P0 * z_channels, f32);
    if ((r = alloc_stream(v, &v->h_in, P0 * (size_t)(ch * ch_mult[n_mult - 1])))) return r;
    DEV_ALLOC(m, alloc, v->y, PH * (size_t)v->conv_out.CoP); DEV_ALLOC(m, alloc, v->idx, P0); DEV_ALLOC(m, alloc, v->dzq, P0 * embed_dim);
    const int ntiles = ceil_div(n_embed, 64);
    DEV_ALLOC(m, alloc, v->pmin, P0 * ntiles); DEV_ALLOC(m, alloc, v->pidx, P0 * ntiles);
    DEV_ALLOC(m, alloc_op, v->a, maxPC, f32);
    DEV_ALLOC(m, alloc_op, v->tA, maxAttnPC, f32); DEV_ALLOC(m, alloc_op, v->tB, maxAttnPC, f32); DEV_ALLOC(m, alloc_op, v->tC, maxAttnPC, f32);
    DEV_ALLOC(m, alloc_op, v->tD, maxAttnPC, f32);
    DEV_ALLOC(m, alloc_op, v->dqkv, maxAttnPC * 3, f32); DEV_ALLOC(m, alloc_op, v->dy8, PH * 8, f32);
    v->dycol = v->Wd_col = nullptr;
    if (!v->f32 && v->conv_out.CoP == 8) {
        const int Cin = v->conv_out.Cin;
        DEV_ALLOC(m, alloc_op, v->dycol, PH * 128, f32); DEV_ALLOC(m, alloc_op, v->Wd_col, (size_t)Cin * 128, f32);
        PRX_CHECK_HIP(hipMemsetAsync(v->Wd_col, 0, (size_t)Cin * 128 * sizeof(bf16_t), s));
        PRX_CHECK_HIP(hipMemcpy2DAsync(v->Wd_col, 128 * sizeof(bf16_t), v->conv_out.Wd, 72 * sizeof(bf16_t), 72 * sizeof(bf16_t), Cin, hipMemcpyDeviceToDevice, s));
    }
    DEV_ALLOC(m, alloc, v->S, maxAttnPC);
    for (void** g : {&v->g0, &v->g1, &v->g2})
        if ((r = alloc_stream(v, g, maxPC))) return r;
    if (v->f32 || v->lean) { v->g0b = v->g0; v->g1b = v->g1; v->g2b = v->g2; }
    else { DEV_ALLOC(m, alloc_op, v->g0b, maxPC, f32); DEV_ALLOC(m, alloc_op, v->g1b, maxPC, f32); DEV_ALLOC(m, alloc_op, v->g2b, maxPC, f32); }
    v->h_in_bf = nullptr;
    for (size_t i = 0; i < v->stages.size(); ++i) {
        const Stage& st = v->stages[i];
        const bool need = (st.kind == 0 && v->res[st.idx].has_sc) || st.kind == 2;
        if (!need) continue;
        void** slot; size_t cnt; void* self;
        if (i == 0) { slot = &v->h_in_bf; cnt = P0 * (size_t)(ch * ch_mult[n_mult - 1]); self = v->h_in; }
        else {
            const Stage& pr = v->stages[i - 1];
            if (pr.kind == 0) { ResBlock& b = v->res[pr.idx]; slot = &b.out_bf; cnt = (size_t)b.rh * b.rw * b.Cout; self = b.out; }
            else if (pr.kind == 1) { AttnBlock& b = v->attn[pr.idx]; slot = &b.out_bf; cnt = (size_t)b.rh * b.rw * b.C; self = b.out; }
            else { UpBlock& b = v->ups[pr.idx]; slot = &b.out_bf; cnt = (size_t)b.rh * b.rw * b.C; self = b.out; }
        }
        if (v->f32 || v->lean) *slot = self;
        else DEV_ALLOC(m, alloc_op, *slot, cnt, f32);
    }
    {
        DEV_ALLOC(m, alloc, v->all_stats, (size_t)2 * v->n_gn * 64);
        auto fix = [&](GN& g) { g.stats = v->all_stats + (size_t)g.id * 64; g.bstats = v->all_stats + (size_t)(v->n_gn + g.id) * 64; };
        for (auto& b : v->res) { fix(b.n1); fix(b.n2); }
        for (auto& b : v->attn) fix(b.n);
        fix(v->norm_out);
    }
    v->ws_bytes = (size_t)64 << 20;
    DEV_ALLOC(m, alloc, v->ws, v->ws_bytes / sizeof(float));
    if (v->h16) DEV_ALLOC(m, alloc, v->gs, 2 + 256);
    *out = guard.release();
    return 0;
}

void prx_vqgan_destroy_impl(PrxVqgan* v) { delete v; }

static bool fusable(const PrxVqgan* v, int C) {
    static const bool f32_fuse = [] { const char* e = getenv("PRX_F32_GN_FUSE"); return !(e && atoi(e) == 0); }();
    const int gs = C / 32;
    return (!v->f32 || f32_fuse) && C % 32 == 0 && gs >= 4 && (gs & (gs - 1)) == 0;
}

static int zero_if_padded(const PrxVqgan* v, void* buf, size_t rows, int P, hipStream_t s) {
    if (pad8(P) != P) PRX_CHECK_HIP(hipMemsetAsync(buf, 0, rows * (size_t)pad8(P) * op_esz(v->f32), s));
    return 0;
}


static void vq_trace(const PrxVqgan* v, const char* tag, int i, const void* p_, size_t n, hipStream_t s) {
    static const bool on = getenv("PRX_VQ_TRACE") != nullptr;
    if (!on || !p_ || v->lean) return;
    const float* p = (const float*)p_;
    std::vector<float> h(n);
    (void)hipStreamSynchronize(s);
    (void)hipMemcpy(h.data(), p, n * sizeof(float), hipMemcpyDeviceToHost);
    double q = 0, mx = 0;
    for (float x : h) { q += (double)x * x; mx = fabs(x) > mx ? fabs(x) : mx; }
    fprintf(stderr, "[vq] %s %2d n=%zu l2 %.9e max %.6e\n", tag, i, n, sqrt(q), mx);
}

static int vg(PrxVqgan* v, GemmDesc& d, hipStream_t s) {
    if (v->f32) {
        d.f32 = 1; d.a_is_f32 = 0;
        if (d.out_bf16 == (void*)d.out_f32) d.out_bf16 = nullptr;
    }
    d.h16 = v->h16;
    return prx_gemm_launch(d, v->ws, v->ws_bytes, s, &v->gctx);
}
GemmCtx* prx_vqgan_gemm_ctx_impl(PrxVqgan* v) { return v ? &v->gctx : nullptr; }

static void out_stream(const PrxVqgan* v, GemmDesc& d, void* stream, int ld, void* twin) {
    if (v->lean) { d.out_bf16 = stream ? stream : twin; d.ldc_bf16 = ld; }
    else { d.out_f32 = (float*)stream; d.ldc_f32 = ld; d.out_bf16 = twin; d.ldc_bf16 = ld; }
}
static void resid_stream(const PrxVqgan* v, GemmDesc& d, const void* r, int ld) {
    if (!r) return;
    d.ldr = ld;
    d.resid = (const float*)r;
    if (v->lean) d.row16 |= 1;
}
static int conv3_fwd(PrxVqgan* v, const Conv3& c, const void* x, bool x_f32, int rh, int rw, bool up, const void* resid,
                     void* out, int ldc, hipStream_t s, void* out_bf = nullptr, const GN* stats_for = nullptr, bool f32_out = false) {
    GemmDesc d; d.A = x; d.a_is_f32 = x_f32; d.a_mode = PRX_A_CONV3X3; d.lda = c.Cin;
    d.B = c.Wf; d.ldb = 9 * c.Cin; d.M = rh * rw; d.N = c.CoP; d.K = 9 * c.Cin;
    d.H = rh; d.W = rw; d.Cin = c.Cin; d.up = up; d.bias_n = c.b;
    resid_stream(v, d, resid, c.Cout);
    if (f32_out) { d.out_f32 = (float*)out; d.ldc_f32 = ldc; }
    else { out_stream(v, d, out, ldc, out_bf); if (!v->lean) d.ldc_bf16 = c.Cout; }
    if (stats_for && stats_for->C == c.Cout && fusable(v, c.Cout)) { d.gn_stats = stats_for->stats; d.gn_gs = c.Cout / 32; }
    return vg(v, d, s);
}
static void set_gnb(const PrxVqgan* v, GemmDesc& d, const GN* gnb, const void* gnb_x, int swish) {
    if (!gnb || !fusable(v, gnb->C) || d.N != gnb->C) return;
    d.gn_stats = gnb->bstats; d.gn_gs = gnb->C / 32;
    d.gnb_x = (const float*)gnb_x;
    if (v->lean) d.row16 |= 2;
    d.gnb_fstats = gnb->stats; d.gnb_gamma = gnb->g; d.gnb_beta = gnb->b; d.gnb_swish = swish; d.gnb_eps = 1e-6f;
}
static int conv3_bwd(PrxVqgan* v, const Conv3& c, const void* dy, bool dy_f32, int rh, int rw, void* dx, hipStream_t s,
                     void* dx_bf = nullptr, const GN* gnb = nullptr, const void* gnb_x = nullptr, int gnb_swish = 1) {
    GemmDesc d; d.A = dy; d.a_is_f32 = dy_f32; d.a_mode = PRX_A_CONV3X3; d.lda = c.CoP;
    d.B = c.Wd; d.ldb = 9 * c.CoP; d.M = rh * rw; d.N = c.Cin; d.K = 9 * c.CoP;
    d.H = rh; d.W = rw; d.Cin = c.CoP; d.up = 0;
    out_stream(v, d, dx, c.Cin, dx_bf);
    set_gnb(v, d, gnb, gnb_x, gnb_swish);
    return vg(v, d, s);
}
static const GN* first_norm(const PrxVqgan* v, int si) {
    if (si >= (int)v->stages.size()) return &v->norm_out;
    const Stage& st = v->stages[si];
    if (st.kind == 0) return &v->res[st.idx].n1;
    if (st.kind == 1) return &v->attn[st.idx].n;
    return nullptr;
}
static int gn_fwd(PrxVqgan* v, const GN& g, const void* x, int P, int swish, hipStream_t s, bool stats_ready = false) {
    return prx_groupnorm_fwd(x, g.g, g.b, g.stats, v->f32 ? nullptr : (bf16_t*)v->a, v->f32 ? (float*)v->a : nullptr, 1, P, g.C, swish,
                             1e-6f, s, 0, stats_ready ? 1 : 0, v->h16, v->lean);
}
static int gn_bwd(PrxVqgan* v, const GN& g, const void* grad, const void* x, const void* add, void* dx,
                  void* dx_bf, int P, int swish, hipStream_t s, bool stats_ready = false) {
    return prx_groupnorm_bwd(grad, x, g.g, g.b, g.stats, g.bstats, add, v->lean ? nullptr : (float*)dx, v->f32 ? nullptr : (bf16_t*)dx_bf, 1, P, g.C,
                             swish, 1e-6f, s, 0, stats_ready && fusable(v, g.C) ? 1 : 0, v->h16, v->lean);
}

int prx_vqgan_bounds_impl(PrxVqgan* v, float* zmin, float* zmax, hipStream_t s) {
    PRX_CHECK_HIP(hipMemcpyAsync(zmin, v->zmin, sizeof(float) * v->D, hipMemcpyDeviceToDevice, s));
    PRX_CHECK_HIP(hipMemcpyAsync(zmax, v->zmax, sizeof(float) * v->D, hipMemcpyDeviceToDevice, s));
    return 0;
}

int prx_vqgan_synth_impl(PrxVqgan* v, const float* z, float* img, int* indices, int quantize, hipStream_t s) {
    const int P0 = v->h0 * v->w0;
    int r;
    PRX_CHECK_HIP(hipMemsetAsync(v->all_stats, 0, sizeof(double) * (size_t)v->n_gn * 64, s));
    if (quantize) {
        if ((r = prx_vq_nearest(z, 1, P0, v->codebook, v->cnorm, P0, v->NC, v->D, v->pmin, v->pidx, v->idx, v->zq, s))) return r;
        if (indices) PRX_CHECK_HIP(hipMemcpyAsync(indices, v->idx, sizeof(int) * P0, hipMemcpyDeviceToDevice, s));
    } else {
        if ((r = prx_nchw_to_nhwc(z, v->zq, nullptr, 1, v->zc, P0, v->zc, s))) return r;
    }
    {   GemmDesc d; d.A = v->zq; d.a_is_f32 = 1; d.lda = v->D; d.B = v->pq.W; d.ldb = v->D; d.M = P0; d.N = v->zc; d.K = v->D;
        d.bias_n = v->pq.b; d.out_bf16 = v->pqo_bf; d.ldc_bf16 = v->zc;
        if ((r = vg(v, d, s))) return r; }
    const GN* nx = first_norm(v, 0);
    if ((r = conv3_fwd(v, v->conv_in, v->pqo_bf, false, v->h0, v->w0, false, nullptr, v->h_in, v->conv_in.Cout, s, v->h_in_bf, nx))) return r;
    bool sr = nx && nx->C == v->conv_in.Cout && fusable(v, nx->C);
    void* x = v->h_in;
    void* x_bf = v->h_in_bf;
    for (int si = 0; si < (int)v->stages.size(); ++si) {
        const Stage& st = v->stages[si];
        nx = first_norm(v, si + 1);
        if (st.kind == 0) {
            ResBlock& b = v->res[st.idx];
            const int P = b.rh * b.rw;
            b.x_in = x; b.x_in_bf = x_bf;
            if ((r = gn_fwd(v, b.n1, x, P, 1, s, sr))) return r;
            if ((r = conv3_fwd(v, b.c1, v->a, false, b.rh, b.rw, false, nullptr, b.h1, b.Cout, s, nullptr, &b.n2))) return r;
            const void* resid = x;
            if (b.has_sc) {
                PRX_REQUIRE(x_bf != nullptr, "vqgan: missing bf16 twin for the shortcut input");
                GemmDesc d; d.A = x_bf; d.lda = b.Cin; d.B = b.sc.W; d.ldb = b.Cin; d.M = P; d.N = b.Cout; d.K = b.Cin;
                d.bias_n = b.sc.b; out_stream(v, d, b.scbuf, b.Cout, nullptr);
                if ((r = vg(v, d, s))) return r;
                resid = b.scbuf;
            }
            if ((r = gn_fwd(v, b.n2, b.h1, P, 1, s, fusable(v, b.Cout)))) return r;
            if ((r = conv3_fwd(v, b.c2, v->a, false, b.rh, b.rw, false, resid, b.out, b.Cout, s, b.out_bf, nx))) return r;
            sr = nx && nx->C == b.Cout && fusable(v, b.Cout);
            x = b.out; x_bf = b.out_bf;
        } else if (st.kind == 1) {
            AttnBlock& b = v->attn[st.idx];
            const int P = b.rh * b.rw, C = b.C;
            b.x_in = x;
            if ((r = gn_fwd(v, b.n, x, P, 0, s, sr))) return r;
            {   GemmDesc d; d.A = v->a; d.lda = C; d.B = b.qkv.W; d.ldb = C; d.M = P; d.N = 3 * C; d.K = C;
                d.bias_n = b.qkv.b; d.out_bf16 = b.qkvb; d.ldc_bf16 = 3 * C;
                if ((r = vg(v, d, s))) return r; }
            const int P8 = pad8(P);
            if ((r = prx_transpose_op(b.qkvb, 3 * C, b.qkvT, P8, P, 3 * C, v->f32, s))) return r;
            {   GemmDesc d; d.A = b.qkvb; d.lda = 3 * C; d.B = op_off(b.qkvb, C, v->f32); d.ldb = 3 * C; d.M = P; d.N = P; d.K = C;
                d.out_f32 = v->S; d.ldc_f32 = P;
                if ((r = vg(v, d, s))) return r; }
            if ((r = prx_softmax_rows(v->S, P, 1.f / sqrtf((float)C), b.Pm, P8, b.PT, P8, P, P, v->prec, s))) return r;
            {   GemmDesc d; d.A = b.Pm; d.lda = P8; d.B = op_off(b.qkvT, (size_t)2 * C * P8, v->f32); d.ldb = P8; d.M = P; d.N = C; d.K = P8;
                d.out_bf16 = v->tB; d.ldc_bf16 = C;
                if ((r = vg(v, d, s))) return r; }
            {   GemmDesc d; d.A = v->tB; d.lda = C; d.B = b.proj.W; d.ldb = C; d.M = P; d.N = C; d.K = C;
                d.bias_n = b.proj.b; resid_stream(v, d, x, C); out_stream(v, d, b.out, C, b.out_bf);
                if (nx && nx->C == C && fusable(v, C)) { d.gn_stats = nx->stats; d.gn_gs = C / 32; }
                if ((r = vg(v, d, s))) return r; }
            sr = nx && nx->C == C && fusable(v, C);
            x = b.out; x_bf = b.out_bf;
        } else {
            UpBlock& b = v->ups[st.idx];
            b.x_in = x; b.x_in_bf = x_bf;
            PRX_REQUIRE(x_bf != nullptr, "vqgan: missing bf16 twin for the upsample input");
            if ((r = conv3_fwd(v, b.c, x_bf, false, b.rh, b.rw, true, nullptr, b.out, b.C, s, b.out_bf, nx))) return r;
            sr = nx && nx->C == b.C && fusable(v, b.C);
            x = b.out; x_bf = b.out_bf;
        }
        {   const int Pq = st.kind == 0 ? v->res[st.idx].rh * v->res[st.idx].rw : st.kind == 1 ? v->attn[st.idx].rh * v->attn[st.idx].rw : v->ups[st.idx].rh * v->ups[st.idx].rw;
            const int Cq = st.kind == 0 ? v->res[st.idx].Cout : st.kind == 1 ? v->attn[st.idx].C : v->ups[st.idx].C;
            vq_trace(v, "fwd", si, x, (size_t)Pq * Cq, s); }
    }
    v->x_last = x;
    const int PH = v->H * v->W;
    if ((r = gn_fwd(v, v->norm_out, x, PH, 1, s, sr))) return r;
    if ((r = conv3_fwd(v, v->conv_out, v->a, false, v->H, v->W, false, nullptr, v->y, v->conv_out.CoP, s, nullptr, nullptr, true))) return r;
    return prx_image_head_fwd(v->y, v->conv_out.CoP, img, 1, v->out_ch, PH, s);
}

long long prx_vqgan_debug_stage_impl(PrxVqgan* v, int stage, float* dst, long long max_floats, hipStream_t s) {
    const void* src = nullptr; long long n = 0;
    PRX_REQUIRE(!v->lean || stage == -2 || stage >= (int)v->stages.size(), "vqgan debug_stage: the stage outputs are 16-bit in the lean layout (PRX_LEAN=0 for fp32 streams)");
    const int ns = (int)v->stages.size();
    if (stage == -2) { src = v->zq; n = (long long)v->h0 * v->w0 * v->D; }
    else if (stage == -1) { src = v->h_in; n = (long long)v->h0 * v->w0 * v->conv_in.Cout; }
    else if (stage >= 0 && stage < ns) {
        const Stage& st = v->stages[stage];
        if (st.kind == 0) { const ResBlock& b = v->res[st.idx]; src = b.out; n = (long long)b.rh * b.rw * b.Cout; }
        else if (st.kind == 1) { const AttnBlock& b = v->attn[st.idx]; src = b.out; n = (long long)b.rh * b.rw * b.C; }
        else { const UpBlock& b = v->ups[st.idx]; src = b.out; n = (long long)b.rh * b.rw * b.C; }
    } else if (stage == ns) { src = v->y; n = (long long)v->H * v->W * v->conv_out.CoP; }
    else if (stage == ns + 1) { src = reinterpret_cast<const float*>(v->all_stats); n = (long long)v->n_gn * 64 * 2; }
    else return -1;
    if (n > max_floats) n = max_floats;
    if (hipMemcpyAsync(dst, src, sizeof(float) * n, hipMemcpyDeviceToDevice, s) != hipSuccess) return -1;
    return n;
}

int prx_vqgan_backward_impl(PrxVqgan* v, const float* g_img, float* dz, hipStream_t s) {
    const int PH = v->H * v->W;
    int r;
    PRX_REQUIRE(v->x_last != nullptr, "vqgan backward: no forward in flight on this handle");
    PRX_CHECK_HIP(hipMemsetAsync(v->all_stats + (size_t)v->n_gn * 64, 0, sizeof(double) * (size_t)v->n_gn * 64, s));
    if (v->h16 && (r = prx_grad_scale(g_img, (size_t)v->out_ch * PH, v->gs + 2, 256, prx_grad_target_log2(), v->gs, s))) return r;
    struct GB { void* f; void* b; };
    GB g{v->g0, v->g0b}, t1{v->g1, v->g1b}, t2{v->g2, v->g2b};
    if (v->dycol) {
        if ((r = prx_image_head_bwd_im2col(v->y, v->conv_out.CoP, g_img, (bf16_t*)v->dycol, 128, v->out_ch, v->H, v->W, s, v->h16, v->gs))) return r;
        GemmDesc d; d.A = v->dycol; d.lda = 128; d.B = v->Wd_col; d.ldb = 128; d.M = PH; d.N = v->conv_out.Cin; d.K = 128;
        out_stream(v, d, t1.f, v->conv_out.Cin, nullptr);
        set_gnb(v, d, &v->norm_out, v->x_last, 1);
        if ((r = vg(v, d, s))) return r;
    } else {
        if ((r = prx_image_head_bwd(v->y, v->conv_out.CoP, g_img, v->f32 ? (float*)v->dy8 : nullptr, v->f32 ? nullptr : (bf16_t*)v->dy8, v->conv_out.CoP, 1,
                                    v->out_ch, PH, s, v->h16, v->gs))) return r;
        if ((r = conv3_bwd(v, v->conv_out, v->dy8, false, v->H, v->W, t1.f, s, nullptr, &v->norm_out, v->x_last, 1))) return r;
    }
    if ((r = gn_bwd(v, v->norm_out, t1.f, v->x_last, nullptr, g.f, g.b, PH, 1, s, true))) return r;
    for (int si = (int)v->stages.size() - 1; si >= 0; --si) {
        const Stage& st = v->stages[si];
        if (st.kind == 0) {
            ResBlock& b = v->res[st.idx];
            const int P = b.rh * b.rw;
            if ((r = conv3_bwd(v, b.c2, g.b, false, b.rh, b.rw, t1.f, s, nullptr, &b.n2, b.h1, 1))) return r;
            if ((r = gn_bwd(v, b.n2, t1.f, b.h1, nullptr, v->f32 ? t2.f : nullptr, t2.b, P, 1, s, true))) return r;
            if ((r = conv3_bwd(v, b.c1, t2.b, false, b.rh, b.rw, t1.f, s, nullptr, &b.n1, b.x_in, 1))) return r;
            const void* add = g.f;
            if (b.has_sc) {
                GemmDesc d; d.A = g.b; d.lda = b.Cout; d.B = b.sc.WT; d.ldb = b.Cout; d.M = P; d.N = b.Cin; d.K = b.Cout;
                out_stream(v, d, t2.f, b.Cin, nullptr);
                if ((r = vg(v, d, s))) return r;
                add = t2.f;
            }
            GB& dst = (add == g.f) ? t2 : g;
            if ((r = gn_bwd(v, b.n1, t1.f, b.x_in, add, dst.f, dst.b, P, 1, s, true))) return r;
            if (&dst != &g) std::swap(g, t2);
        } else if (st.kind == 1) {
            AttnBlock& b = v->attn[st.idx];
            const int P = b.rh * b.rw, C = b.C;
            {   GemmDesc d; d.A = g.b; d.lda = C; d.B = b.proj.WT; d.ldb = C; d.M = P; d.N = C; d.K = C;
                d.out_bf16 = v->tA; d.ldc_bf16 = C;
                if ((r = vg(v, d, s))) return r; }
            {   GemmDesc d; d.A = v->tA; d.lda = C; d.B = op_off(b.qkvb, 2 * C, v->f32); d.ldb = 3 * C; d.M = P; d.N = P; d.K = C;
                d.out_f32 = v->S; d.ldc_f32 = P;
                if ((r = vg(v, d, s))) return r; }
            const int P8 = pad8(P);
            if ((r = zero_if_padded(v, v->tB, P, P, s))) return r;
            if ((r = zero_if_padded(v, v->tC, P, P, s))) return r;
            if ((r = prx_softmax_rows_bwd(b.Pm, P8, v->S, P, 1.f / sqrtf((float)C), v->tB, P8, v->tC, P8, P, P, v->prec, s))) return r;
            {   GemmDesc d; d.A = v->tB; d.lda = P8; d.B = op_off(b.qkvT, (size_t)C * P8, v->f32); d.ldb = P8; d.M = P; d.N = C; d.K = P8;
                d.out_bf16 = v->dqkv; d.ldc_bf16 = 3 * C;
                if ((r = vg(v, d, s))) return r; }
            {   GemmDesc d; d.A = v->tC; d.lda = P8; d.B = b.qkvT; d.ldb = P8; d.M = P; d.N = C; d.K = P8;
                d.out_bf16 = op_off(v->dqkv, C, v->f32); d.ldc_bf16 = 3 * C;
                if ((r = vg(v, d, s))) return r; }
            if ((r = zero_if_padded(v, v->tD, C, P, s))) return r;
            if ((r = prx_transpose_op(v->tA, C, v->tD, P8, P, C, v->f32, s))) return r;
            {   GemmDesc d; d.A = b.PT; d.lda = P8; d.B = v->tD; d.ldb = P8; d.M = P; d.N = C; d.K = P8;
                d.out_bf16 = op_off(v->dqkv, 2 * C, v->f32); d.ldc_bf16 = 3 * C;
                if ((r = vg(v, d, s))) return r; }
            {   GemmDesc d; d.A = v->dqkv; d.lda = 3 * C; d.B = b.qkv.WT; d.ldb = 3 * C; d.M = P; d.N = C; d.K = 3 * C;
                out_stream(v, d, t1.f, C, nullptr);
                set_gnb(v, d, &b.n, b.x_in, 0);
                if ((r = vg(v, d, s))) return r; }
            if ((r = gn_bwd(v, b.n, t1.f, b.x_in, g.f, t2.f, t2.b, P, 0, s, true))) return r;
            std::swap(g, t2);
        } else {
            UpBlock& b = v->ups[st.idx];
            if ((r = conv3_bwd(v, b.c, g.b, false, b.rh, b.rw, t1.f, s))) return r;
            if ((r = prx_upsample2x_bwd(t1.f, v->lean ? nullptr : (float*)t2.f, v->f32 ? nullptr : (bf16_t*)t2.b, 1, b.rh / 2, b.rw / 2, b.C, s, v->h16,
                                        v->lean))) return r;
            std::swap(g, t2);
        }
        {   const int Pq = st.kind == 0 ? v->res[st.idx].rh * v->res[st.idx].rw : st.kind == 1 ? v->attn[st.idx].rh * v->attn[st.idx].rw : v->ups[st.idx].rh * v->ups[st.idx].rw / 4;
            const int Cq = st.kind == 0 ? v->res[st.idx].Cin : st.kind == 1 ? v->attn[st.idx].C : v->ups[st.idx].C;
            vq_trace(v, "bwd", si, g.f, (size_t)Pq * Cq, s); }
    }
    if ((r = conv3_bwd(v, v->conv_in, g.b, false, v->h0, v->w0, v->lean ? nullptr : t1.f, s, v->dpq_bf))) return r;
    const int P0 = v->h0 * v->w0;
    {   GemmDesc d; d.A = v->dpq_bf; d.lda = v->zc; d.B = v->pq.WT; d.ldb = v->zc; d.M = P0; d.N = v->D; d.K = v->zc;
        d.out_f32 = v->dzq; d.ldc_f32 = v->D;
        if (v->h16) d.alpha_dev = v->gs + 1;
        if ((r = vg(v, d, s))) return r; }
    return prx_nhwc_to_nchw(v->dzq, v->D, dz, 1, v->D, P0, s);
}
```

Baseline: 165.7.

## Fuse grad-scale reduction, add optional fused image head, merge stats memsets

Merges the two-kernel fp16 gradient-scale reduction into one kernel that uses a last-block ticket to do the final reduction, removing a launch. Adds an env-gated fused GroupNorm+swish+3x3 conv image-head forward and backward kernel that replaces the GEMM-based output conv. Also merges the forward and backward GroupNorm stats memsets into one, and writes VQ indices directly instead of copying them. The fused head is off unless PRX_VQ_HEAD_FUSED is set. The ticket counter relies on atomicInc wrapping back to zero so it resets between calls.

```diff
diff --git a/pixray_amd/csrc/common.h b/pixray_amd/csrc/common.h
--- a/pixray_amd/csrc/common.h
+++ b/pixray_amd/csrc/common.h
@@ -160,6 +160,13 @@
 
 __device__ __forceinline__ float sigmoidf_(float x) { return 1.f / (1.f + __expf(-x)); }
 
+__device__ __forceinline__ void part_publish(float* p, float v) { __hip_atomic_store(p, v, __ATOMIC_RELAXED, __HIP_MEMORY_SCOPE_AGENT); }
+__device__ __forceinline__ float part_read(const float* p) { return __hip_atomic_load(p, __ATOMIC_RELAXED, __HIP_MEMORY_SCOPE_AGENT); }
+__device__ __forceinline__ bool part_last_ticket(unsigned* ticket) {
+    asm volatile("s_waitcnt vmcnt(0)" ::: "memory");
+    return atomicInc(ticket, gridDim.x - 1) == gridDim.x - 1;
+}
+
 __device__ __forceinline__ unsigned xcd_linear(unsigned bid, unsigned nwg) {
     const unsigned xcd = bid & 7u, local = bid >> 3, q = nwg >> 3, r = nwg & 7u;
     return (xcd < r ? xcd * (q + 1) : r * (q + 1) + (xcd - r) * q) + local;
diff --git a/pixray_amd/csrc/elementwise.h b/pixray_amd/csrc/elementwise.h
--- a/pixray_amd/csrc/elementwise.h
+++ b/pixray_amd/csrc/elementwise.h
@@ -13,7 +13,8 @@
                        int HW, hipStream_t s, int h16 = 0, const float* gscale = nullptr);
 int prx_image_head_bwd_im2col(const float* x, int ldc, const float* gimg, bf16_t* col, int ldk, int C, int H, int W, hipStream_t s, int h16 = 0,
                               const float* gscale = nullptr);
-int prx_grad_scale(const float* g, size_t n, float* part, int nparts, int target_log2, float* scale2, hipStream_t s);
+int prx_grad_scale(const float* g, size_t n, float* part, int nparts, int target_log2, float* scale2, hipStream_t s,
+                   unsigned* ticket = nullptr);
 int prx_adam_clamp(float* z, float* m, float* v, const float* g, const float* zmin, const float* zmax, int hw,
                    size_t n, float lr, float b1, float b2, float eps, int step, hipStream_t s);
 int prx_adam_clamp_dev(float* z, float* m, float* v, const float* g, const float* zmin, const float* zmax, int hw,
diff --git a/pixray_amd/csrc/elementwise.hip b/pixray_amd/csrc/elementwise.hip
--- a/pixray_amd/csrc/elementwise.hip
+++ b/pixray_amd/csrc/elementwise.hip
@@ -231,12 +231,11 @@
     __syncthreads();
     if (threadIdx.x == 0) part[blockIdx.x] = fmaxf(fmaxf(s[0], s[1]), fmaxf(s[2], s[3]));
 }
-__global__ __launch_bounds__(256) void grad_scale_final_kernel(const float* __restrict__ part, int nparts, int target_log2,
-                                                               float* __restrict__ scale2) {
+template <bool SHARED>
+__device__ __forceinline__ void grad_scale_final(const float* part, int nparts, int target_log2, float* __restrict__ scale2, float* s) {
     float m = 0.f;
-    for (int i = threadIdx.x; i < nparts; i += blockDim.x) m = fmaxf(m, part[i]);
+    for (int i = threadIdx.x; i < nparts; i += blockDim.x) m = fmaxf(m, SHARED ? part_read(part + i) : part[i]);
     m = wave_max(m);
-    __shared__ float s[4];
     if ((threadIdx.x & 63) == 0) s[threadIdx.x >> 6] = m;
     __syncthreads();
     if (threadIdx.x == 0) {
@@ -253,6 +252,32 @@
         scale2[1] = 1.f / S;
     }
 }
+__global__ __launch_bounds__(256) void grad_scale_final_kernel(const float* __restrict__ part, int nparts, int target_log2,
+                                                               float* __restrict__ scale2) {
+    __shared__ float s[4];
+    grad_scale_final<false>(part, nparts, target_log2, scale2, s);
+}
+__device__ unsigned grad_scale_ticket = 0;
+__global__ __launch_bounds__(256) void grad_scale_kernel(const float* __restrict__ g, size_t n, float* part, int target_log2,
+                                                         float* __restrict__ scale2, unsigned* __restrict__ ticket) {
+    float m = 0.f;
+    for (size_t i = (size_t)blockIdx.x * blockDim.x + threadIdx.x; i < n; i += (size_t)gridDim.x * blockDim.x) {
+        const float a = fabsf(g[i]);
+        m = fmaxf(m, a == a ? a : INFINITY);
+    }
+    m = wave_max(m);
+    __shared__ float s[4];
+    __shared__ unsigned last;
+    if ((threadIdx.x & 63) == 0) s[threadIdx.x >> 6] = m;
+    __syncthreads();
+    if (threadIdx.x == 0) {
+        part_publish(part + blockIdx.x, fmaxf(fmaxf(s[0], s[1]), fmaxf(s[2], s[3])));
+        last = part_last_ticket(ticket ? ticket : &grad_scale_ticket) ? 1u : 0u;
+    }
+    __syncthreads();
+    if (!last) return;
+    grad_scale_final<true>(part, (int)gridDim.x, target_log2, scale2, s);
+}
 
 __global__ __launch_bounds__(256) void scale_dev_kernel(float* __restrict__ x, size_t n, const float* __restrict__ scale, bf16_t* __restrict__ out16, int h16) {
     const float sc = *scale;
@@ -322,12 +347,10 @@
     PRX_LAUNCH_CHECK();
     return 0;
 }
-int prx_grad_scale(const float* g, size_t n, float* part, int nparts, int target_log2, float* scale2, hipStream_t s) {
+int prx_grad_scale(const float* g, size_t n, float* part, int nparts, int target_log2, float* scale2, hipStream_t s, unsigned* ticket) {
     PRX_REQUIRE(nparts >= 1 && nparts <= 1024, "grad_scale: 1..1024 partials");
     const int blocks = (int)std::min<size_t>((n + 1023) / 1024 + 1, (size_t)nparts);
-    hipLaunchKernelGGL(amax_partial_kernel, dim3(blocks), dim3(256), 0, s, g, n, part);
-    PRX_LAUNCH_CHECK();
-    hipLaunchKernelGGL(grad_scale_final_kernel, dim3(1), dim3(256), 0, s, part, blocks, target_log2, scale2);
+    hipLaunchKernelGGL(grad_scale_kernel, dim3(blocks), dim3(256), 0, s, g, n, part, target_log2, scale2, ticket);
     PRX_LAUNCH_CHECK();
     return 0;
 }
diff --git a/pixray_amd/csrc/image_head.h b/pixray_amd/csrc/image_head.h
--- /dev/null
+++ b/pixray_amd/csrc/image_head.h
@@ -0,0 +1,15 @@
+#pragma once
+#include "common.h"
+
+#define PRX_HEAD_C 128
+
+static inline bool prx_head_fused_ok(int C, int out_ch, int CoP, int H, int W) {
+    return C == PRX_HEAD_C && out_ch >= 1 && out_ch <= 4 && CoP == 8 && H >= 1 && W >= 1 &&
+           (unsigned long long)H * W * PRX_HEAD_C < (1ull << 31);
+}
+int prx_head_pack(const void* Wf, int out_ch, float* wfw, float* wbw, hipStream_t s);
+int prx_head_fused_fwd(const void* x, const double* fstats, const float* gamma, const float* beta, const float* wfw, const float* bias,
+                       float* y, float* img, int H, int W, int out_ch, float eps, hipStream_t s);
+int prx_head_fused_bwd(const void* x, const double* fstats, double* bstats, const float* gamma, const float* beta, const float* wbw,
+                       const float* y, const float* gimg, const float* gscale, void* dx, int H, int W, int out_ch, float eps,
+                       hipStream_t s);
diff --git a/pixray_amd/csrc/image_head.hip b/pixray_amd/csrc/image_head.hip
--- /dev/null
+++ b/pixray_amd/csrc/image_head.hip
@@ -0,0 +1,243 @@
+#include "image_head.h"
+
+namespace {
+
+constexpr int HC_ = PRX_HEAD_C;
+constexpr int TH = 8, TW = 16;
+constexpr int HROWS = TH + 2, HCOLS = TW + 2, NPX = HROWS * HCOLS;
+constexpr int PITCH = HC_ + 8;
+
+__device__ __forceinline__ void head_mean_rstd(const double* st, double n, float eps, float& mean, float& rstd) {
+    double m = st[0] / n;
+    double var = st[1] / n - m * m;
+    if (var < 0) var = 0;
+    mean = (float)m;
+    rstd = (float)(1.0 / sqrt(var + (double)eps));
+}
+__device__ __forceinline__ float head_swish_grad(float y) {
+    float s = sigmoidf_(y);
+    return s * (1.f + y * (1.f - s));
+}
+
+__global__ __launch_bounds__(256) void head_pack_kernel(const half_t* __restrict__ Wf, int out_ch, float* __restrict__ wfw,
+                                                        float* __restrict__ wbw) {
+    const int i = blockIdx.x * blockDim.x + threadIdx.x;
+    if (i >= 9 * HC_ * out_ch) return;
+    const int co = i % out_ch, c = (i / out_ch) % HC_, tap = (i / out_ch) / HC_;
+    const float w = (float)Wf[(size_t)co * 9 * HC_ + tap * HC_ + c];
+    wfw[(tap * HC_ + c) * out_ch + co] = w;
+    wbw[(c * 9 + tap) * out_ch + co] = w;
+}
+
+template <int NCO>
+__global__ __launch_bounds__(256) void head_fwd_kernel(const half_t* __restrict__ x, const double* __restrict__ fstats,
+                                                       const float* __restrict__ gamma, const float* __restrict__ beta,
+                                                       const float* __restrict__ wfw, const float* __restrict__ bias,
+                                                       float* __restrict__ y, float* __restrict__ img, int H, int W, float eps) {
+    __shared__ __attribute__((aligned(16))) half_t tile[NPX * PITCH];
+    __shared__ float smr[32][2];
+    __shared__ float red[128][4];
+    const int tid = threadIdx.x;
+    const int tiles_x = (W + TW - 1) / TW;
+    const int x0 = (int)(blockIdx.x % tiles_x) * TW, y0 = (int)(blockIdx.x / tiles_x) * TH;
+    if (tid < 32) {
+        float m, r;
+        head_mean_rstd(fstats + tid * 2, (double)H * W * (HC_ / 32), eps, m, r);
+        smr[tid][0] = m; smr[tid][1] = r;
+    }
+    __syncthreads();
+    {
+        const int c8 = tid & 15;
+        const float4 g0 = reinterpret_cast<const float4*>(gamma)[c8 * 2], g1 = reinterpret_cast<const float4*>(gamma)[c8 * 2 + 1];
+        const float4 b0 = reinterpret_cast<const float4*>(beta)[c8 * 2], b1 = reinterpret_cast<const float4*>(beta)[c8 * 2 + 1];
+        const float ga[8] = {g0.x, g0.y, g0.z, g0.w, g1.x, g1.y, g1.z, g1.w}, be[8] = {b0.x, b0.y, b0.z, b0.w, b1.x, b1.y, b1.z, b1.w};
+        const float mean[2] = {smr[c8 * 2][0], smr[c8 * 2 + 1][0]}, rstd[2] = {smr[c8 * 2][1], smr[c8 * 2 + 1][1]};
+        for (int i = tid; i < NPX * 16; i += 256) {
+            const int px = i >> 4, hy = px / HCOLS, hx = px - hy * HCOLS;
+            const int gy = y0 + hy - 1, gx = x0 + hx - 1;
+            f16x8 o;
+#pragma unroll
+            for (int j = 0; j < 8; ++j) o[j] = (half_t)0.f;
+            if (gy >= 0 && gy < H && gx >= 0 && gx < W) {
+                const f16x8 v = *reinterpret_cast<const f16x8*>(x + (unsigned)(gy * W + gx) * HC_ + c8 * 8);
+#pragma unroll
+                for (int j = 0; j < 8; ++j) {
+                    const float yv = ((float)v[j] - mean[j >> 2]) * rstd[j >> 2] * ga[j] + be[j];
+                    o[j] = f32_to_f16_sat(yv * sigmoidf_(yv));
+                }
+            }
+            *reinterpret_cast<f16x8*>(tile + px * PITCH + c8 * 8) = o;
+        }
+    }
+    __syncthreads();
+    const int pix = tid & 127, py = pix >> 4, pxx = pix & 15;
+    const int hf = __builtin_amdgcn_readfirstlane(tid >> 7);
+    float acc[NCO];
+#pragma unroll
+    for (int co = 0; co < NCO; ++co) acc[co] = 0.f;
+#pragma unroll
+    for (int tap = 0; tap < 9; ++tap) {
+        const half_t* row = tile + ((py + tap / 3) * HCOLS + pxx + tap % 3) * PITCH + hf * 64;
+        const float* wt = wfw + (tap * HC_ + hf * 64) * NCO;
+#pragma unroll
+        for (int c8 = 0; c8 < 8; ++c8) {
+            const f16x8 v = *reinterpret_cast<const f16x8*>(row + c8 * 8);
+#pragma unroll
+            for (int j = 0; j < 8; ++j) {
+                const float xv = (float)v[j];
+#pragma unroll
+                for (int co = 0; co < NCO; ++co) acc[co] = fmaf(xv, wt[(c8 * 8 + j) * NCO + co], acc[co]);
+            }
+        }
+    }
+    if (hf == 1) {
+#pragma unroll
+        for (int co = 0; co < NCO; ++co) red[pix][co] = acc[co];
+    }
+    __syncthreads();
+    const int gy = y0 + py, gx = x0 + pxx;
+    if (hf == 0 && gy < H && gx < W) {
+        const unsigned p = (unsigned)(gy * W + gx), HWp = (unsigned)(H * W);
+        float o[8] = {0.f, 0.f, 0.f, 0.f, 0.f, 0.f, 0.f, 0.f};
+#pragma unroll
+        for (int co = 0; co < NCO; ++co) {
+            o[co] = (acc[co] + red[pix][co]) + bias[co];
+            const float u = (o[co] + 1.f) * 0.5f;
+            img[co * HWp + p] = fminf(fmaxf(u, 0.f), 1.f);
+        }
+        reinterpret_cast<float4*>(y)[p * 2] = make_float4(o[0], o[1], o[2], o[3]);
+        reinterpret_cast<float4*>(y)[p * 2 + 1] = make_float4(o[4], o[5], o[6], o[7]);
+    }
+}
+
+template <int NCO, bool APPLY>
+__global__ __launch_bounds__(1024) void head_bwd_kernel(const half_t* __restrict__ x, const double* __restrict__ fstats,
+                                                        double* __restrict__ bstats, const float* __restrict__ gamma,
+                                                        const float* __restrict__ beta, const float* __restrict__ wbw,
+                                                        const float* __restrict__ y, const float* __restrict__ gimg,
+                                                        const float* __restrict__ gscale_dev, half_t* __restrict__ dx, int H, int W,
+                                                        float eps) {
+    __shared__ float smr[32][4];
+    __shared__ double wsum[16][16];
+    const int tid = threadIdx.x, lane = tid & 63, pl = tid & 255;
+    const int wave = __builtin_amdgcn_readfirstlane(tid >> 6), quarter = wave >> 2;
+    const int HWp = H * W;
+    if (tid < 32) {
+        const double n = (double)HWp * (HC_ / 32);
+        float m, r;
+        head_mean_rstd(fstats + tid * 2, n, eps, m, r);
+        smr[tid][0] = m; smr[tid][1] = r;
+        smr[tid][2] = APPLY ? (float)(bstats[tid * 2] / n) : 0.f;
+        smr[tid][3] = APPLY ? (float)(bstats[tid * 2 + 1] / n) : 0.f;
+    }
+    if (!APPLY && tid < 256) (&wsum[0][0])[tid] = 0.0;
+    __syncthreads();
+    const float gscale = gscale_dev ? *gscale_dev : 1.f;
+    for (int q0 = (int)blockIdx.x * 256; q0 < HWp; q0 += (int)gridDim.x * 256) {
+        const int q = q0 + pl;
+        const bool valid = q < HWp;
+        const int qc = valid ? q : HWp - 1;
+        const int qy = qc / W, qx = qc - qy * W;
+        float dyv[9][NCO];
+#pragma unroll
+        for (int tap = 0; tap < 9; ++tap) {
+            const int yy = qy + 1 - tap / 3, xx = qx + 1 - tap % 3;
+            const bool inb = valid && yy >= 0 && yy < H && xx >= 0 && xx < W;
+            const unsigned r = inb ? (unsigned)(yy * W + xx) : (unsigned)qc;
+#pragma unroll
+            for (int co = 0; co < NCO; ++co) {
+                const float u = (y[r * 8 + co] + 1.f) * 0.5f;
+                const float g = gimg[(unsigned)co * (unsigned)HWp + r];
+                const float uc = fminf(fmaxf(u, 0.f), 1.f);
+                const float d = (g * (u - uc) >= 0.f) ? (0.5f * gscale) * g : 0.f;
+                dyv[tap][co] = inb ? d : 0.f;
+            }
+        }
+#pragma unroll 1
+        for (int k = 0; k < 4; ++k) {
+            const f16x8 xv = *reinterpret_cast<const f16x8*>(x + (unsigned)qc * HC_ + quarter * 32 + k * 8);
+            float o[8], s[2][2] = {{0.f, 0.f}, {0.f, 0.f}};
+#pragma unroll
+            for (int j = 0; j < 8; ++j) {
+                const int c = quarter * 32 + k * 8 + j, grp = c >> 2;
+                const float* w = wbw + c * (9 * NCO);
+                float da = 0.f;
+#pragma unroll
+                for (int tap = 0; tap < 9; ++tap)
+#pragma unroll
+                    for (int co = 0; co < NCO; ++co) da = fmaf(dyv[tap][co], w[tap * NCO + co], da);
+                const float mean = smr[grp][0], rstd = smr[grp][1], gam = gamma[c];
+                const float xh = ((float)xv[j] - mean) * rstd;
+                const float dxh = da * head_swish_grad(xh * gam + beta[c]) * gam;
+                if (APPLY) o[j] = rstd * (dxh - smr[grp][2] - xh * smr[grp][3]);
+                else { s[j >> 2][0] += dxh; s[j >> 2][1] += dxh * xh; }
+            }
+            if (APPLY) {
+                if (valid) {
+                    f16x8 h;
+#pragma unroll
+                    for (int j = 0; j < 8; ++j) h[j] = f32_to_f16_sat(o[j]);
+                    *reinterpret_cast<f16x8*>(dx + (unsigned)q * HC_ + quarter * 32 + k * 8) = h;
+                }
+            } else {
+#pragma unroll
+                for (int gg = 0; gg < 2; ++gg)
+#pragma unroll
+                    for (int m = 0; m < 2; ++m) {
+                        const float t = wave_sum(valid ? s[gg][m] : 0.f);
+                        if (lane == 0) wsum[wave][(k * 2 + gg) * 2 + m] += (double)t;
+                    }
+            }
+        }
+    }
+    if (!APPLY) {
+        __syncthreads();
+        if (tid < 64) {
+            const int grp = tid >> 1, m = tid & 1, qd = grp >> 3, lg = grp & 7;
+            double t = 0.0;
+            for (int w4 = 0; w4 < 4; ++w4) t += wsum[qd * 4 + w4][lg * 2 + m];
+            atomicAdd(&bstats[grp * 2 + m], t);
+        }
+    }
+}
+
+}
+
+#define HEAD_NCO_DISPATCH(nco, ...)                                               \
+    do {                                                                          \
+        switch (nco) {                                                            \
+            case 1: { constexpr int NCO = 1; __VA_ARGS__; } break;                \
+            case 2: { constexpr int NCO = 2; __VA_ARGS__; } break;                \
+            case 3: { constexpr int NCO = 3; __VA_ARGS__; } break;                \
+            default: { constexpr int NCO = 4; __VA_ARGS__; } break;               \
+        }                                                                         \
+    } while (0)
+
+int prx_head_pack(const void* Wf, int out_ch, float* wfw, float* wbw, hipStream_t s) {
+    PRX_REQUIRE(Wf && wfw && wbw && out_ch >= 1 && out_ch <= 4, "image head: bad weight pack arguments");
+    hipLaunchKernelGGL(head_pack_kernel, dim3(ceil_div(9 * HC_ * 4, 256)), dim3(256), 0, s, (const half_t*)Wf, out_ch, wfw, wbw);
+    PRX_LAUNCH_CHECK();
+    return 0;
+}
+int prx_head_fused_fwd(const void* x, const double* fstats, const float* gamma, const float* beta, const float* wfw, const float* bias,
+                       float* y, float* img, int H, int W, int out_ch, float eps, hipStream_t s) {
+    PRX_REQUIRE(prx_head_fused_ok(HC_, out_ch, 8, H, W), "image head: %d x %d x %d channels out is not a layer of the fused head", H, W, out_ch);
+    const int blocks = ceil_div(W, TW) * ceil_div(H, TH);
+    HEAD_NCO_DISPATCH(out_ch, hipLaunchKernelGGL(head_fwd_kernel<NCO>, dim3(blocks), dim3(256), 0, s, (const half_t*)x, fstats, gamma, beta,
+                                                 wfw, bias, y, img, H, W, eps));
+    PRX_LAUNCH_CHECK();
+    return 0;
+}
+int prx_head_fused_bwd(const void* x, const double* fstats, double* bstats, const float* gamma, const float* beta, const float* wbw,
+                       const float* y, const float* gimg, const float* gscale, void* dx, int H, int W, int out_ch, float eps,
+                       hipStream_t s) {
+    PRX_REQUIRE(prx_head_fused_ok(HC_, out_ch, 8, H, W), "image head: %d x %d x %d channels out is not a layer of the fused head", H, W, out_ch);
+    const int blocks = ceil_div(H * W, 256);
+    HEAD_NCO_DISPATCH(out_ch, hipLaunchKernelGGL((head_bwd_kernel<NCO, false>), dim3(std::min(blocks, 256)), dim3(1024), 0, s, (const half_t*)x,
+                                                 fstats, bstats, gamma, beta, wbw, y, gimg, gscale, (half_t*)dx, H, W, eps));
+    PRX_LAUNCH_CHECK();
+    HEAD_NCO_DISPATCH(out_ch, hipLaunchKernelGGL((head_bwd_kernel<NCO, true>), dim3(blocks), dim3(1024), 0, s, (const half_t*)x,
+                                                 fstats, bstats, gamma, beta, wbw, y, gimg, gscale, (half_t*)dx, H, W, eps));
+    PRX_LAUNCH_CHECK();
+    return 0;
+}
diff --git a/pixray_amd/csrc/resnet.hip b/pixray_amd/csrc/resnet.hip
--- a/pixray_amd/csrc/resnet.hip
+++ b/pixray_amd/csrc/resnet.hip
@@ -475,7 +475,10 @@
     if (r->lean) { DEV_ALLOC(m, alloc_op, r->gb2, maxMC, f32); DEV_ALLOC(m, alloc_op, r->gb3, maxMC, f32); } else DEV_ALLOC(m, alloc, r->gB, maxMC);
     DEV_ALLOC(m, alloc_op, r->tb1, maxMC, f32); DEV_ALLOC(m, alloc_op, r->tb2, maxMC, f32); DEV_ALLOC(m, alloc_op, r->gbf, maxMC, f32);
     DEV_ALLOC(m, alloc, r->dY, N * 3 * (size_t)res * res); DEV_ALLOC(m, alloc, r->mm_part, 2 * 1024);
-    if (r->h16) DEV_ALLOC(m, alloc, r->gs, 2 + 64);
+    if (r->h16) {
+        DEV_ALLOC(m, alloc, r->gs, 2 + 64);
+        PRX_CHECK_HIP(hipMemsetAsync(r->gs + 2 + 63, 0, sizeof(unsigned), s));
+    }
     r->ws_bytes = (size_t)64 << 20;
     DEV_ALLOC(m, alloc, r->ws, r->ws_bytes / sizeof(float));
     *out = guard.release();
@@ -543,7 +546,7 @@
     {   GemmDesc d; d.A = r->de; d.a_is_f32 = 1; d.lda = r->out_dim; d.B = r->WcT; d.ldb = r->out_dim; d.M = n; d.N = C; d.K = r->out_dim;
         d.out_bf16 = r->do0; d.ldc_bf16 = C;
         if (r->h16) {
-            if ((e = prx_grad_scale(r->de, (size_t)n * r->out_dim, r->gs + 2, 64, prx_grad_target_log2(), r->gs, s))) return e;
+            if ((e = prx_grad_scale(r->de, (size_t)n * r->out_dim, r->gs + 2, 63, prx_grad_target_log2(), r->gs, s, reinterpret_cast<unsigned*>(r->gs + 2 + 63)))) return e;
             if ((e = prx_scale_dev(r->de, (size_t)n * r->out_dim, r->gs, s))) return e;
         }
         if ((e = rg(r, d, s))) return e; }
diff --git a/pixray_amd/csrc/vit.hip b/pixray_amd/csrc/vit.hip
--- a/pixray_amd/csrc/vit.hip
+++ b/pixray_amd/csrc/vit.hip
@@ -273,7 +273,10 @@
     if (v->f32) { v->dx_bf = v->dx; v->dh_bf = v->dh; }
     else { DEV_ALLOC(m, alloc_op, v->dx_bf, R * W, f32); DEV_ALLOC(m, alloc_op, v->dh_bf, R * W, f32); }
     DEV_ALLOC(m, alloc, v->dhpost, (size_t)max_n * W); DEV_ALLOC(m, alloc, v->mm_part, 2 * 1024);
-    if (v->h16) DEV_ALLOC(m, alloc, v->gs, 2 + 64);
+    if (v->h16) {
+        DEV_ALLOC(m, alloc, v->gs, 2 + 64);
+        PRX_CHECK_HIP(hipMemsetAsync(v->gs + 2 + 63, 0, sizeof(unsigned), s));
+    }
     v->ws_bytes = (size_t)64 << 20;
     DEV_ALLOC(m, alloc, v->ws, v->ws_bytes / sizeof(float));
     *out = guard.release();
@@ -384,7 +387,7 @@
     {   GemmDesc d; d.A = v->de; d.a_is_f32 = 1; d.lda = v->out_dim; d.B = v->proj; d.ldb = v->out_dim;
         d.M = n; d.N = W; d.K = v->out_dim; d.out_f32 = v->dhpost; d.ldc_f32 = W;
         if (v->h16) {
-            if ((r = prx_grad_scale(v->de, (size_t)n * v->out_dim, v->gs + 2, 64, prx_grad_target_log2(), v->gs, s))) return r;
+            if ((r = prx_grad_scale(v->de, (size_t)n * v->out_dim, v->gs + 2, 63, prx_grad_target_log2(), v->gs, s, reinterpret_cast<unsigned*>(v->gs + 2 + 63)))) return r;
             if ((r = prx_scale_dev(v->de, (size_t)n * v->out_dim, v->gs, s, (bf16_t*)v->de16, v->h16))) return r;
             d.A = v->de16; d.a_is_f32 = 0;
         }
diff --git a/pixray_amd/csrc/vqgan.hip b/pixray_amd/csrc/vqgan.hip
--- a/pixray_amd/csrc/vqgan.hip
+++ b/pixray_amd/csrc/vqgan.hip
@@ -8,6 +8,7 @@
 #include <vector>
 #include <memory>
 #include <stdlib.h>
+#include "image_head.h"
 
 namespace {
 
@@ -100,8 +101,10 @@
     void *g0, *g1, *g2;
     void *g0b, *g1b, *g2b;
     double* all_stats; int n_gn;
+    bool bstats_clear;
     float* ws; size_t ws_bytes;
     void* x_last;
+    int head_fused; float *head_wf, *head_wb;
 };
 
 namespace {
@@ -272,6 +275,13 @@
         PRX_CHECK_HIP(hipMemsetAsync(v->Wd_col, 0, (size_t)Cin * 128 * sizeof(bf16_t), s));
         PRX_CHECK_HIP(hipMemcpy2DAsync(v->Wd_col, 128 * sizeof(bf16_t), v->conv_out.Wd, 72 * sizeof(bf16_t), 72 * sizeof(bf16_t), Cin, hipMemcpyDeviceToDevice, s));
     }
+    {   const char* e = getenv("PRX_VQ_HEAD_FUSED");
+        v->head_fused = v->lean && e && atoi(e) != 0 && prx_head_fused_ok(v->conv_out.Cin, out_ch, v->conv_out.CoP, rh, rw) ? 1 : 0;
+        v->head_wf = v->head_wb = nullptr;
+        if (v->head_fused) {
+            DEV_ALLOC(m, alloc, v->head_wf, (size_t)9 * PRX_HEAD_C * 4); DEV_ALLOC(m, alloc, v->head_wb, (size_t)9 * PRX_HEAD_C * 4);
+            if ((r = prx_head_pack(v->conv_out.Wf, out_ch, v->head_wf, v->head_wb, s))) return r;
+        } }
     DEV_ALLOC(m, alloc, v->S, maxAttnPC);
     for (void** g : {&v->g0, &v->g1, &v->g2})
         if ((r = alloc_stream(v, g, maxPC))) return r;
@@ -302,7 +312,11 @@
     }
     v->ws_bytes = (size_t)64 << 20;
     DEV_ALLOC(m, alloc, v->ws, v->ws_bytes / sizeof(float));
-    if (v->h16) DEV_ALLOC(m, alloc, v->gs, 2 + 256);
+    if (v->h16) {
+        DEV_ALLOC(m, alloc, v->gs, 2 + 256);
+        PRX_CHECK_HIP(hipMemsetAsync(v->gs + 2 + 255, 0, sizeof(unsigned), s));
+    }
+    v->bstats_clear = false;
     *out = guard.release();
     return 0;
 }
@@ -406,10 +420,10 @@
 int prx_vqgan_synth_impl(PrxVqgan* v, const float* z, float* img, int* indices, int quantize, hipStream_t s) {
     const int P0 = v->h0 * v->w0;
     int r;
-    PRX_CHECK_HIP(hipMemsetAsync(v->all_stats, 0, sizeof(double) * (size_t)v->n_gn * 64, s));
+    PRX_CHECK_HIP(hipMemsetAsync(v->all_stats, 0, sizeof(double) * (size_t)2 * v->n_gn * 64, s));
+    v->bstats_clear = true;
     if (quantize) {
-        if ((r = prx_vq_nearest(z, 1, P0, v->codebook, v->cnorm, P0, v->NC, v->D, v->pmin, v->pidx, v->idx, v->zq, s))) return r;
-        if (indices) PRX_CHECK_HIP(hipMemcpyAsync(indices, v->idx, sizeof(int) * P0, hipMemcpyDeviceToDevice, s));
+        if ((r = prx_vq_nearest(z, 1, P0, v->codebook, v->cnorm, P0, v->NC, v->D, v->pmin, v->pidx, indices ? indices : v->idx, v->zq, s))) return r;
     } else {
         if ((r = prx_nchw_to_nhwc(z, v->zq, nullptr, 1, v->zc, P0, v->zc, s))) return r;
     }
@@ -479,6 +493,12 @@
     }
     v->x_last = x;
     const int PH = v->H * v->W;
+    if (v->head_fused) {
+        if (!sr && (r = prx_groupnorm_fwd(x, v->norm_out.g, v->norm_out.b, v->norm_out.stats, nullptr, nullptr, 1, PH, v->norm_out.C, 1, 1e-6f, s,
+                                          0, 0, v->h16, v->lean))) return r;
+        return prx_head_fused_fwd(x, v->norm_out.stats, v->norm_out.g, v->norm_out.b, v->head_wf, v->conv_out.b, v->y, img, v->H, v->W, v->out_ch,
+                                  1e-6f, s);
+    }
     if ((r = gn_fwd(v, v->norm_out, x, PH, 1, s, sr))) return r;
     if ((r = conv3_fwd(v, v->conv_out, v->a, false, v->H, v->W, false, nullptr, v->y, v->conv_out.CoP, s, nullptr, nullptr, true))) return r;
     return prx_image_head_fwd(v->y, v->conv_out.CoP, img, 1, v->out_ch, PH, s);
@@ -486,8 +506,8 @@
 
 long long prx_vqgan_debug_stage_impl(PrxVqgan* v, int stage, float* dst, long long max_floats, hipStream_t s) {
     const void* src = nullptr; long long n = 0;
-    PRX_REQUIRE(!v->lean || stage == -2 || stage >= (int)v->stages.size(), "vqgan debug_stage: the stage outputs are 16-bit in the lean layout (PRX_LEAN=0 for fp32 streams)");
     const int ns = (int)v->stages.size();
+    const bool s16 = v->lean && stage >= -1 && stage < ns;
     if (stage == -2) { src = v->zq; n = (long long)v->h0 * v->w0 * v->D; }
     else if (stage == -1) { src = v->h_in; n = (long long)v->h0 * v->w0 * v->conv_in.Cout; }
     else if (stage >= 0 && stage < ns) {
@@ -498,8 +518,8 @@
     } else if (stage == ns) { src = v->y; n = (long long)v->H * v->W * v->conv_out.CoP; }
     else if (stage == ns + 1) { src = reinterpret_cast<const float*>(v->all_stats); n = (long long)v->n_gn * 64 * 2; }
     else return -1;
-    if (n > max_floats) n = max_floats;
-    if (hipMemcpyAsync(dst, src, sizeof(float) * n, hipMemcpyDeviceToDevice, s) != hipSuccess) return -1;
+    if (n > (s16 ? 2 * max_floats : max_floats)) n = s16 ? 2 * max_floats : max_floats;
+    if (hipMemcpyAsync(dst, src, (s16 ? sizeof(bf16_t) : sizeof(float)) * n, hipMemcpyDeviceToDevice, s) != hipSuccess) return -1;
     return n;
 }
 
@@ -507,11 +527,15 @@
     const int PH = v->H * v->W;
     int r;
     PRX_REQUIRE(v->x_last != nullptr, "vqgan backward: no forward in flight on this handle");
-    PRX_CHECK_HIP(hipMemsetAsync(v->all_stats + (size_t)v->n_gn * 64, 0, sizeof(double) * (size_t)v->n_gn * 64, s));
-    if (v->h16 && (r = prx_grad_scale(g_img, (size_t)v->out_ch * PH, v->gs + 2, 256, prx_grad_target_log2(), v->gs, s))) return r;
+    if (!v->bstats_clear) PRX_CHECK_HIP(hipMemsetAsync(v->all_stats + (size_t)v->n_gn * 64, 0, sizeof(double) * (size_t)v->n_gn * 64, s));
+    v->bstats_clear = false;
+    if (v->h16 && (r = prx_grad_scale(g_img, (size_t)v->out_ch * PH, v->gs + 2, 255, prx_grad_target_log2(), v->gs, s, reinterpret_cast<unsigned*>(v->gs + 2 + 255)))) return r;
     struct GB { void* f; void* b; };
     GB g{v->g0, v->g0b}, t1{v->g1, v->g1b}, t2{v->g2, v->g2b};
-    if (v->dycol) {
+    if (v->head_fused) {
+        if ((r = prx_head_fused_bwd(v->x_last, v->norm_out.stats, v->norm_out.bstats, v->norm_out.g, v->norm_out.b, v->head_wb, v->y, g_img, v->gs,
+                                    g.b, v->H, v->W, v->out_ch, 1e-6f, s))) return r;
+    } else if (v->dycol) {
         if ((r = prx_image_head_bwd_im2col(v->y, v->conv_out.CoP, g_img, (bf16_t*)v->dycol, 128, v->out_ch, v->H, v->W, s, v->h16, v->gs))) return r;
         GemmDesc d; d.A = v->dycol; d.lda = 128; d.B = v->Wd_col; d.ldb = 128; d.M = PH; d.N = v->conv_out.Cin; d.K = 128;
         out_stream(v, d, t1.f, v->conv_out.Cin, nullptr);
@@ -522,7 +546,7 @@
                                     v->out_ch, PH, s, v->h16, v->gs))) return r;
         if ((r = conv3_bwd(v, v->conv_out, v->dy8, false, v->H, v->W, t1.f, s, nullptr, &v->norm_out, v->x_last, 1))) return r;
     }
-    if ((r = gn_bwd(v, v->norm_out, t1.f, v->x_last, nullptr, g.f, g.b, PH, 1, s, true))) return r;
+    if (!v->head_fused && (r = gn_bwd(v, v->norm_out, t1.f, v->x_last, nullptr, g.f, g.b, PH, 1, s, true))) return r;
     for (int si = (int)v->stages.size() - 1; si >= 0; --si) {
         const Stage& st = v->stages[si];
         if (st.kind == 0) {
```

Measured after the change: 165.8 (median of 3 runs). About the same (+0.1%).
